# alasdairtran/transform-and-tell

Measured on AMD Instinct MI355X. Metric: training samples/sec (img+article->caption), higher is better.
Workload: dtype bf16; 1 GPU; BASELINE configs[2] (= per-GPU shape of configs[3]): expt/nytimes/9_transformer_objects - full faces+objects model (4 contexts: ResNet-152 image regions, RoBERTa-large article with the 25-layer weigh_bert mix, 4 faces, 64 objects), batch 32/GPU, 512-token articles, 32 caption steps; full step = frozen encoders fwd + decoder fwd/loss/bwd + BertAdam; global_batch=32, article_len=512, caption_len=33, parallelism=dp1, step_graph_replays=188, skipped_steps=0

## Files before the change

transform-and-tell_amd/csrc/common.h:

```cpp
#pragma once
#include <hip/hip_runtime.h>
#include <stdint.h>

#define TELL_OK 0
#define TELL_ERR_ARG (-1)
#define TELL_ERR_LAUNCH (-2)

#define TELL_F32 0
#define TELL_BF16 1

typedef __bf16 bf16_t;
typedef __attribute__((ext_vector_type(8))) __bf16 bf16x8;
typedef __attribute__((ext_vector_type(4))) float f32x4;
typedef __attribute__((ext_vector_type(16))) float f32x16;

extern "C" void tell_set_error(const char* msg);

static inline int tell_check_launch(const char* what) {
  hipError_t e = hipGetLastError();
  if (e != hipSuccess) {
    tell_set_error(hipGetErrorString(e));
    (void)what;
    return TELL_ERR_LAUNCH;
  }
  return TELL_OK;
}

#define TELL_REQUIRE(cond, msg)  \
  do {                           \
    if (!(cond)) {               \
      tell_set_error(msg);       \
      return TELL_ERR_ARG;       \
    }                            \
  } while (0)

__device__ __forceinline__ float bf2f(uint16_t b) { return __uint_as_float(((uint32_t)b) << 16); }
__device__ __forceinline__ uint16_t f2bf(float f) {
  uint32_t u = __float_as_uint(f);
  if ((u & 0x7fffffffu) > 0x7f800000u) return (uint16_t)((u >> 16) | 0x40u);
  u += 0x7fffu + ((u >> 16) & 1u);
  return (uint16_t)(u >> 16);
}

__device__ __forceinline__ float tell_glu(float a, float g) { return a * __builtin_amdgcn_rcpf(1.f + __expf(-g)); }

template <typename T> struct Elem;
template <> struct Elem<float> {
  static constexpr int VEC = 4;
  __device__ static __forceinline__ float ld(const float* p) { return *p; }
  __device__ static __forceinline__ void st(float* p, float v) { *p = v; }
};
template <> struct Elem<uint16_t> {
  static constexpr int VEC = 8;
  __device__ static __forceinline__ float ld(const uint16_t* p) { return bf2f(*p); }
  __device__ static __forceinline__ void st(uint16_t* p, float v) { *p = f2bf(v); }
};

__device__ __forceinline__ void unpack16(const uint4& c, float (&v)[4], const float*) {
  v[0] = __uint_as_float(c.x); v[1] = __uint_as_float(c.y);
  v[2] = __uint_as_float(c.z); v[3] = __uint_as_float(c.w);
}
__device__ __forceinline__ void unpack16(const uint4& c, float (&v)[8], const uint16_t*) {
  v[0] = __uint_as_float(c.x << 16); v[1] = __uint_as_float(c.x & 0xffff0000u);
  v[2] = __uint_as_float(c.y << 16); v[3] = __uint_as_float(c.y & 0xffff0000u);
  v[4] = __uint_as_float(c.z << 16); v[5] = __uint_as_float(c.z & 0xffff0000u);
  v[6] = __uint_as_float(c.w << 16); v[7] = __uint_as_float(c.w & 0xffff0000u);
}
__device__ __forceinline__ uint4 pack16(const float (&v)[4], const float*) {
  return make_uint4(__float_as_uint(v[0]), __float_as_uint(v[1]), __float_as_uint(v[2]),
                    __float_as_uint(v[3]));
}
__device__ __forceinline__ uint4 pack16(const float (&v)[8], const uint16_t*) {
  return make_uint4((uint32_t)f2bf(v[0]) | ((uint32_t)f2bf(v[1]) << 16),
                    (uint32_t)f2bf(v[2]) | ((uint32_t)f2bf(v[3]) << 16),
                    (uint32_t)f2bf(v[4]) | ((uint32_t)f2bf(v[5]) << 16),
                    (uint32_t)f2bf(v[6]) | ((uint32_t)f2bf(v[7]) << 16));
}

__device__ __forceinline__ float wave_sum(float v) {
#pragma unroll
  for (int o = 32; o > 0; o >>= 1) v += __shfl_xor(v, o, 64);
  return v;
}
__device__ __forceinline__ float wave_max(float v) {
#pragma unroll
  for (int o = 32; o > 0; o >>= 1) v = fmaxf(v, __shfl_xor(v, o, 64));
  return v;
}

extern const uint32_t* g_tell_rng_step;
extern const uint32_t* g_tell_pos_step;
extern uint32_t* g_tell_pos_next;
__device__ __forceinline__ uint32_t tell_step_salt(uint32_t salt, const uint32_t* step) {
  return step ? salt + *step * 0x632BE5ABu : salt;
}

__device__ __host__ __forceinline__ uint32_t tell_quad_x(uint32_t seed, uint64_t quad) {
  return (uint32_t)quad * 0x9E3779B1u + seed * 0x85EBCA6Bu;
}
__device__ __host__ __forceinline__ uint32_t tell_quad_y(uint32_t salt, uint64_t quad) {
  return (uint32_t)(quad >> 32) * 0x85EBCA77u + salt * 0xC2B2AE3Du + 0x27D4EB2Fu;
}
__device__ __host__ __forceinline__ uint32_t tell_quad_mix(uint32_t x, uint32_t y) {
  x ^= y; x ^= x >> 16; x *= 0x7FEB352Du; x ^= x >> 15;
  return x;
}
__device__ __host__ __forceinline__ uint32_t tell_quad_a(uint32_t h) {
  const uint32_t a = (h & 0xffffffu) * 0xD1B54Bu;
  return a ^ (a >> 15);
}
__device__ __host__ __forceinline__ uint32_t tell_quad_b(uint32_t h) {
  const uint32_t b = (h >> 8) * 0xA54FF5u;
  return b ^ (b >> 15);
}
__device__ __host__ __forceinline__ uint32_t tell_keep_field(uint32_t seed, uint32_t salt, uint64_t idx) {
  const uint64_t quad = idx >> 2;
  const uint32_t h = tell_quad_mix(tell_quad_x(seed, quad), tell_quad_y(salt, quad));
  const uint32_t w = (idx & 2) ? tell_quad_b(h) : tell_quad_a(h);
  return (idx & 1) ? (w >> 16) : (w & 0xffffu);
}
__device__ __host__ __forceinline__ uint32_t tell_drop_threshold(float p) {
  double t = (double)p * 65536.0;
  if (t < 0) t = 0;
  if (t > 65535.0) t = 65535.0;
  return (uint32_t)t;
}
__device__ __forceinline__ float tell_keep(uint32_t seed, uint32_t salt, uint64_t idx, uint32_t thr,
                                           float inv_keep) {
  return tell_keep_field(seed, salt, idx) >= thr ? inv_keep : 0.f;
}
__device__ __forceinline__ void tell_keep2(uint32_t seed, uint32_t salt, uint64_t idx_even, uint32_t thr,
                                           float inv_keep, float& k0, float& k1) {
  const uint64_t quad = idx_even >> 2;
  const uint32_t h = tell_quad_mix(tell_quad_x(seed, quad), tell_quad_y(salt, quad));
  const uint32_t w = (idx_even & 2) ? tell_quad_b(h) : tell_quad_a(h);
  k0 = (w & 0xffffu) >= thr ? inv_keep : 0.f;
  k1 = (w >> 16) >= thr ? inv_keep : 0.f;
}
struct TellKeepRow { uint32_t x0, y; };
#define TELL_QUAD_STRIDE 0x9E3779B1u
__device__ __forceinline__ bool tell_keep_row_ok(uint64_t quad0, uint32_t span) {
  return (uint32_t)quad0 <= 0xFFFFFFFFu - span;
}
__device__ __forceinline__ TellKeepRow tell_keep_row(uint32_t seed, uint32_t salt, uint64_t quad0) {
  TellKeepRow r;
  r.x0 = tell_quad_x(seed, quad0);
  r.y = tell_quad_y(salt, quad0);
  return r;
}
__device__ __forceinline__ void tell_keep4_bits(uint32_t x, uint32_t y, uint32_t thr, bool& k0, bool& k1, bool& k2,
                                                bool& k3) {
  const uint32_t h = tell_quad_mix(x, y);
  const uint32_t a = tell_quad_a(h), b = tell_quad_b(h);
  k0 = (a & 0xffffu) >= thr;
  k1 = (a >> 16) >= thr;
  k2 = (b & 0xffffu) >= thr;
  k3 = (b >> 16) >= thr;
}

__device__ __host__ __forceinline__ uint32_t tell_sample_bits(uint32_t seed, uint32_t row, uint32_t step) {
  const uint32_t h = tell_quad_mix(tell_quad_x(seed, row), tell_quad_y(step, row));
  return tell_quad_mix(h, 0x27D4EB2Fu);
}
__device__ __host__ __forceinline__ float tell_sample_u(uint32_t seed, uint32_t row, uint32_t step) {
  return (float)(tell_sample_bits(seed, row, step) >> 8) * (1.0f / 16777216.0f);
}
__device__ __host__ __forceinline__ int tell_sample_pick(const float* lp, int k, float inv_temp, float u) {
  const float l0 = lp[0];
  float c = 0.f;
  for (int j = 0; j < k; ++j) c += expf((lp[j] - l0) * inv_temp);
  const float t = u * c;
  float r = 0.f;
  for (int j = 0; j < k; ++j) {
    r += expf((lp[j] - l0) * inv_temp);
    if (t < r) return j;
  }
  return k - 1;
}
```

transform-and-tell_amd/csrc/elementwise.hip:

```cpp
#include "common.h"
#include "gemm_common.h"

static inline int grid_for(long work, int per_block) {
  long g = (work + per_block - 1) / per_block;
  if (g < 1) g = 1;
  if (g > 256 * 16) g = 256 * 16;
  return (int)g;
}

template <typename S, typename D>
__global__ void cast_kernel(const S* __restrict__ src, D* __restrict__ dst, long n) {
  long i = (long)blockIdx.x * blockDim.x + threadIdx.x;
  const long stride = (long)gridDim.x * blockDim.x;
  for (; i < n; i += stride) Elem<D>::st(dst + i, Elem<S>::ld(src + i));
}

extern "C" int tell_cast(const void* src, int src_dtype, void* dst, int dst_dtype, long n,
                         hipStream_t stream) {
  if (n <= 0) return TELL_OK;
  int g = grid_for(n, 256 * 4);
  if (src_dtype == TELL_F32 && dst_dtype == TELL_BF16)
    hipLaunchKernelGGL((cast_kernel<float, uint16_t>), dim3(g), dim3(256), 0, stream, (const float*)src, (uint16_t*)dst, n);
  else if (src_dtype == TELL_BF16 && dst_dtype == TELL_F32)
    hipLaunchKernelGGL((cast_kernel<uint16_t, float>), dim3(g), dim3(256), 0, stream, (const uint16_t*)src, (float*)dst, n);
  else if (src_dtype == TELL_F32 && dst_dtype == TELL_F32)
    hipLaunchKernelGGL((cast_kernel<float, float>), dim3(g), dim3(256), 0, stream, (const float*)src, (float*)dst, n);
  else if (src_dtype == TELL_BF16 && dst_dtype == TELL_BF16)
    hipLaunchKernelGGL((cast_kernel<uint16_t, uint16_t>), dim3(g), dim3(256), 0, stream, (const uint16_t*)src, (uint16_t*)dst, n);
  else { tell_set_error("cast: bad dtype"); return TELL_ERR_ARG; }
  return tell_check_launch("cast");
}

template <typename D>
__global__ __launch_bounds__(256) void scale_cast_kernel(const float* __restrict__ src, D* __restrict__ dst, long n,
                                                         const float* __restrict__ scale) {
  const float sc = scale ? *scale : 1.f;
  const long nv = n / 4;
  for (long i = (long)blockIdx.x * blockDim.x + threadIdx.x; i < nv; i += (long)gridDim.x * blockDim.x) {
    const float4 v = reinterpret_cast<const float4*>(src)[i];
    Elem<D>::st(dst + 4 * i, v.x * sc); Elem<D>::st(dst + 4 * i + 1, v.y * sc);
    Elem<D>::st(dst + 4 * i + 2, v.z * sc); Elem<D>::st(dst + 4 * i + 3, v.w * sc);
  }
  if (blockIdx.x == 0 && threadIdx.x < (n & 3)) Elem<D>::st(dst + nv * 4 + threadIdx.x, src[nv * 4 + threadIdx.x] * sc);
}
extern "C" int tell_scale_cast(const float* src, void* dst, int dst_dtype, long n, const float* scale_dev,
                               hipStream_t stream) {
  if (n <= 0) return TELL_OK;
  TELL_REQUIRE(((uintptr_t)src & 15) == 0, "scale_cast: src must be 16-byte aligned");
  int g = grid_for(n / 4 + 1, 256 * 2);
  if (dst_dtype == TELL_BF16) hipLaunchKernelGGL((scale_cast_kernel<uint16_t>), dim3(g), dim3(256), 0, stream, src, (uint16_t*)dst, n, scale_dev);
  else hipLaunchKernelGGL((scale_cast_kernel<float>), dim3(g), dim3(256), 0, stream, src, (float*)dst, n, scale_dev);
  return tell_check_launch("scale_cast");
}

template <typename S, typename D>
__global__ __launch_bounds__(256) void transpose_kernel(const S* __restrict__ src, long ld_src,
                                                        D* __restrict__ dst_t, long ld_t,
                                                        D* __restrict__ dst_plain, long ld_p,
                                                        const float* __restrict__ row_scale,
                                                        int rows, int cols) {
  __shared__ float tile[64][65];
  const int r0 = blockIdx.y * 64, c0 = blockIdx.x * 64;
  const int tx = threadIdx.x & 63, ty = threadIdx.x >> 6;
  for (int i = ty; i < 64; i += 4) {
    int r = r0 + i, c = c0 + tx;
    float v = 0.f;
    if (r < rows && c < cols) {
      v = Elem<S>::ld(src + (long)r * ld_src + c);
      if (row_scale) v *= row_scale[r];
      if (dst_plain) Elem<D>::st(dst_plain + (long)r * ld_p + c, v);
    }
    tile[i][tx] = v;
  }
  __syncthreads();
  if (dst_t) {
    for (int i = ty; i < 64; i += 4) {
      int c = c0 + i, r = r0 + tx;
      if (r < rows && c < cols) Elem<D>::st(dst_t + (long)c * ld_t + r, tile[tx][i]);
    }
  }
}

extern "C" int tell_transpose(const void* src, long ld_src, int src_dtype, void* dst_t, long ld_t,
                              void* dst_plain, long ld_p, int dst_dtype, const float* row_scale,
                              int rows, int cols, hipStream_t stream) {
  if (rows <= 0 || cols <= 0) return TELL_OK;
  dim3 grid((cols + 63) / 64, (rows + 63) / 64);
#define TL(S, D) hipLaunchKernelGGL((transpose_kernel<S, D>), grid, dim3(256), 0, stream, (const S*)src, ld_src, \
                                    (D*)dst_t, ld_t, (D*)dst_plain, ld_p, row_scale, rows, cols)
  if (src_dtype == TELL_F32 && dst_dtype == TELL_F32) TL(float, float);
  else if (src_dtype == TELL_F32 && dst_dtype == TELL_BF16) TL(float, uint16_t);
  else if (src_dtype == TELL_BF16 && dst_dtype == TELL_BF16) TL(uint16_t, uint16_t);
  else if (src_dtype == TELL_BF16 && dst_dtype == TELL_F32) TL(uint16_t, float);
  else { tell_set_error("transpose: bad dtype"); return TELL_ERR_ARG; }
#undef TL
  return tell_check_launch("transpose");
}

__global__ __launch_bounds__(256) void wn_rowscale_kernel(const float* __restrict__ g,
                                                          const float* __restrict__ v, int rows,
                                                          int cols, float* __restrict__ scale,
                                                          float* __restrict__ norms) {
  const int lane = threadIdx.x & 63;
  const int row = blockIdx.x * 4 + (threadIdx.x >> 6);
  if (row >= rows) return;
  const float* vr = v + (long)row * cols;
  float s = 0.f;
  for (int c = lane; c < cols; c += 64) { float x = vr[c]; s += x * x; }
  s = wave_sum(s);
  if (lane == 0) {
    float nrm = sqrtf(s);
    norms[row] = nrm;
    scale[row] = g[row] / nrm;
  }
}

extern "C" int tell_wn_rowscale(const float* g, const float* v, int rows, int cols, float* scale,
                                float* norms, hipStream_t stream) {
  if (rows <= 0) return TELL_OK;
  hipLaunchKernelGGL(wn_rowscale_kernel, dim3((rows + 3) / 4), dim3(256), 0, stream, g, v, rows, cols, scale, norms);
  return tell_check_launch("wn_rowscale");
}

template <typename OutT>
__device__ __forceinline__ void wn_weight_row(const float* __restrict__ g, const float* __restrict__ v, int row,
                                              int cols, OutT* __restrict__ w, float* __restrict__ norms, int lane) {
  const float* vr = v + (long)row * cols;
  OutT* wr = w + (long)row * cols;
  float s = 0.f;
  typedef __attribute__((ext_vector_type(4))) float f4v;
  if ((cols & 255) == 0 && cols <= 4096) {
    const int nv = cols >> 8;
    f4v x[16];
#pragma unroll
    for (int j = 0; j < 16; ++j)
      if (j < nv) x[j] = __builtin_nontemporal_load(reinterpret_cast<const f4v*>(vr) + lane + 64 * j);
#pragma unroll
    for (int j = 0; j < 16; ++j)
      if (j < nv) s += x[j][0] * x[j][0] + x[j][1] * x[j][1] + x[j][2] * x[j][2] + x[j][3] * x[j][3];
    s = wave_sum(s);
    const float nrm = sqrtf(s), sc = g[row] / nrm;
    if (lane == 0) norms[row] = nrm;
#pragma unroll
    for (int j = 0; j < 16; ++j)
      if (j < nv) {
        const int c = lane + 64 * j;
        if constexpr (sizeof(OutT) == 2) {
          uint2 o;
          o.x = (uint32_t)f2bf(x[j][0] * sc) | ((uint32_t)f2bf(x[j][1] * sc) << 16);
          o.y = (uint32_t)f2bf(x[j][2] * sc) | ((uint32_t)f2bf(x[j][3] * sc) << 16);
          reinterpret_cast<uint2*>(wr)[c] = o;
        } else {
          reinterpret_cast<float4*>(wr)[c] = make_float4(x[j][0] * sc, x[j][1] * sc, x[j][2] * sc, x[j][3] * sc);
        }
      }
    return;
  }
  if ((cols & 3) == 0) {
    const float4* v4 = reinterpret_cast<const float4*>(vr);
    for (int c = lane; c < cols / 4; c += 64) { const float4 x = v4[c]; s += x.x * x.x + x.y * x.y + x.z * x.z + x.w * x.w; }
  } else {
    for (int c = lane; c < cols; c += 64) { const float x = vr[c]; s += x * x; }
  }
  s = wave_sum(s);
  const float nrm = sqrtf(s), sc = g[row] / nrm;
  if (lane == 0) norms[row] = nrm;
  if ((cols & 3) == 0) {
    const float4* v4 = reinterpret_cast<const float4*>(vr);
    for (int c = lane; c < cols / 4; c += 64) {
      const float4 x = v4[c];
      if constexpr (sizeof(OutT) == 2) {
        uint2 o;
        o.x = (uint32_t)f2bf(x.x * sc) | ((uint32_t)f2bf(x.y * sc) << 16);
        o.y = (uint32_t)f2bf(x.z * sc) | ((uint32_t)f2bf(x.w * sc) << 16);
        reinterpret_cast<uint2*>(wr)[c] = o;
      } else {
        reinterpret_cast<float4*>(wr)[c] = make_float4(x.x * sc, x.y * sc, x.z * sc, x.w * sc);
      }
    }
  } else {
    for (int c = lane; c < cols; c += 64) Elem<OutT>::st(wr + c, vr[c] * sc);
  }
}
template <typename OutT>
__global__ __launch_bounds__(256) void wn_weight_kernel(const float* __restrict__ g, const float* __restrict__ v,
                                                        int rows, int cols, OutT* __restrict__ w,
                                                        float* __restrict__ norms) {
  const int row = blockIdx.x * 4 + (threadIdx.x >> 6);
  if (row < rows) wn_weight_row<OutT>(g, v, row, cols, w, norms, threadIdx.x & 63);
}
extern "C" int tell_wn_weight(const float* g, const float* v, int rows, int cols, void* w, int out_dtype,
                              float* norms, hipStream_t stream) {
  if (rows <= 0) return TELL_OK;
  TELL_REQUIRE(((uintptr_t)v & 15) == 0 && ((uintptr_t)w & 15) == 0, "wn_weight: buffers must be 16-byte aligned");
  if (out_dtype == TELL_BF16)
    hipLaunchKernelGGL((wn_weight_kernel<uint16_t>), dim3((rows + 3) / 4), dim3(256), 0, stream, g, v, rows, cols, (uint16_t*)w, norms);
  else
    hipLaunchKernelGGL((wn_weight_kernel<float>), dim3((rows + 3) / 4), dim3(256), 0, stream, g, v, rows, cols, (float*)w, norms);
  return tell_check_launch("wn_weight");
}

__device__ __forceinline__ void wn_backward_row(const float* __restrict__ dW, const float* __restrict__ g,
                                                const float* __restrict__ v, const float* __restrict__ norms,
                                                int row, int cols, float* __restrict__ dg, float* __restrict__ dv,
                                                int lane, const bool store = false) {
  const float* vr = v + (long)row * cols;
  const float* dr = dW + (long)row * cols;
  float* o = dv + (long)row * cols;
  const bool vec = (cols & 3) == 0 && (((uintptr_t)dW | (uintptr_t)v | (uintptr_t)dv) & 15) == 0;
  float dot = 0.f;
  if (vec && (cols & 255) == 0 && cols <= 4096) {
    typedef __attribute__((ext_vector_type(4))) float f4v;
    const int nv = cols >> 8;
    f4v d[16], x[16];
#pragma unroll
    for (int j = 0; j < 16; ++j)
      if (j < nv) {
        d[j] = __builtin_nontemporal_load(reinterpret_cast<const f4v*>(dr) + lane + 64 * j);
        x[j] = reinterpret_cast<const f4v*>(vr)[lane + 64 * j];
      }
#pragma unroll
    for (int j = 0; j < 16; ++j)
      if (j < nv) dot += d[j][0] * x[j][0] + d[j][1] * x[j][1] + d[j][2] * x[j][2] + d[j][3] * x[j][3];
    dot = wave_sum(dot);
    const float nrm = norms[row], gs = g[row] / nrm, k = dot / (nrm * nrm);
    if (lane == 0) dg[row] = (store ? 0.f : dg[row]) + dot / nrm;
#pragma unroll
    for (int j = 0; j < 16; ++j)
      if (j < nv) {
        const int c = lane + 64 * j;
        float4 a = make_float4(0.f, 0.f, 0.f, 0.f);
        if (!store) a = reinterpret_cast<float4*>(o)[c];
        a.x += gs * (d[j][0] - x[j][0] * k); a.y += gs * (d[j][1] - x[j][1] * k);
        a.z += gs * (d[j][2] - x[j][2] * k); a.w += gs * (d[j][3] - x[j][3] * k);
        reinterpret_cast<float4*>(o)[c] = a;
      }
    return;
  }
  if (vec) {
    for (int c = lane; c < cols / 4; c += 64) {
      const float4 d = reinterpret_cast<const float4*>(dr)[c], x = reinterpret_cast<const float4*>(vr)[c];
      dot += d.x * x.x + d.y * x.y + d.z * x.z + d.w * x.w;
    }
  } else {
    for (int c = lane; c < cols; c += 64) dot += dr[c] * vr[c];
  }
  dot = wave_sum(dot);
  const float nrm = norms[row], gs = g[row] / nrm, k = dot / (nrm * nrm);
  if (lane == 0) dg[row] = (store ? 0.f : dg[row]) + dot / nrm;
  if (vec) {
    for (int c = lane; c < cols / 4; c += 64) {
      const float4 d = reinterpret_cast<const float4*>(dr)[c], x = reinterpret_cast<const float4*>(vr)[c];
      float4 a = make_float4(0.f, 0.f, 0.f, 0.f);
      if (!store) a = reinterpret_cast<float4*>(o)[c];
      a.x += gs * (d.x - x.x * k); a.y += gs * (d.y - x.y * k); a.z += gs * (d.z - x.z * k); a.w += gs * (d.w - x.w * k);
      reinterpret_cast<float4*>(o)[c] = a;
    }
  } else {
    for (int c = lane; c < cols; c += 64) o[c] = (store ? 0.f : o[c]) + gs * (dr[c] - vr[c] * k);
  }
}
__global__ __launch_bounds__(256) void wn_backward_kernel(const float* __restrict__ dW,
                                                          const float* __restrict__ g,
                                                          const float* __restrict__ v,
                                                          const float* __restrict__ norms, int rows,
                                                          int cols, float* __restrict__ dg,
                                                          float* __restrict__ dv) {
  const int row = blockIdx.x * 4 + (threadIdx.x >> 6);
  if (row < rows) wn_backward_row(dW, g, v, norms, row, cols, dg, dv, threadIdx.x & 63);
}

extern "C" int tell_wn_backward(const float* dW, const float* g, const float* v, const float* norms,
                                int rows, int cols, float* dg, float* dv, hipStream_t stream) {
  if (rows <= 0) return TELL_OK;
  hipLaunchKernelGGL(wn_backward_kernel, dim3((rows + 3) / 4), dim3(256), 0, stream, dW, g, v, norms, rows, cols, dg, dv);
  return tell_check_launch("wn_backward");
}

#define WN_MULTI_MAX 32
struct WNMulti {
  const float* a[WN_MULTI_MAX];
  const float* g[WN_MULTI_MAX];
  const float* v[WN_MULTI_MAX];
  void* w[WN_MULTI_MAX];
  float* norms[WN_MULTI_MAX];
  float* dg[WN_MULTI_MAX];
  int cols[WN_MULTI_MAX];
  int row_start[WN_MULTI_MAX + 1];
  int n;
  unsigned store;
};
template <typename OutT, bool BWD>
__global__ __launch_bounds__(256) void wn_multi_kernel(WNMulti m) {
  const int row = blockIdx.x * 4 + (threadIdx.x >> 6), lane = threadIdx.x & 63;
  if (row >= m.row_start[m.n]) return;
  int i = 0;
  while (i + 1 < m.n && row >= m.row_start[i + 1]) ++i;
  const int r = row - m.row_start[i];
  if constexpr (BWD) wn_backward_row(m.a[i], m.g[i], m.v[i], m.norms[i], r, m.cols[i], m.dg[i], static_cast<float*>(m.w[i]), lane, (m.store >> i) & 1u);
  else wn_weight_row<OutT>(m.g[i], m.v[i], r, m.cols[i], static_cast<OutT*>(m.w[i]), m.norms[i], lane);
}
template <bool BWD>
static int wn_multi_launch(int n, const void* const* a, const void* const* g, const void* const* v, void* const* w,
                           void* const* norms, void* const* dg, const int* rows, const int* cols, int out_dtype,
                           hipStream_t stream, const int* store = nullptr) {
  static_assert(WN_MULTI_MAX <= 32, "WNMulti::store is one bit per tensor");
  for (int base = 0; base < n; base += WN_MULTI_MAX) {
    WNMulti m;
    m.n = n - base < WN_MULTI_MAX ? n - base : WN_MULTI_MAX;
    m.row_start[0] = 0;
    m.store = 0u;
    for (int i = 0; i < m.n; ++i) {
      const int j = base + i;
      TELL_REQUIRE(rows[j] > 0 && cols[j] > 0, "wn_multi: empty tensor");
      TELL_REQUIRE(BWD || (((uintptr_t)v[j] | (uintptr_t)w[j]) & 15) == 0, "wn_weight_multi: buffers must be 16-byte aligned");
      m.a[i] = BWD ? static_cast<const float*>(a[j]) : nullptr;
      m.g[i] = static_cast<const float*>(g[j]);
      m.v[i] = static_cast<const float*>(v[j]);
      m.w[i] = w[j];
      m.norms[i] = static_cast<float*>(norms[j]);
      m.dg[i] = BWD ? static_cast<float*>(dg[j]) : nullptr;
      m.cols[i] = cols[j];
      m.row_start[i + 1] = m.row_start[i] + rows[j];
      if (BWD && store && store[j]) m.store |= 1u << i;
    }
    const dim3 grid((m.row_start[m.n] + 3) / 4);
    if (BWD) hipLaunchKernelGGL((wn_multi_kernel<float, true>), grid, dim3(256), 0, stream, m);
    else if (out_dtype == TELL_BF16) hipLaunchKernelGGL((wn_multi_kernel<uint16_t, false>), grid, dim3(256), 0, stream, m);
    else hipLaunchKernelGGL((wn_multi_kernel<float, false>), grid, dim3(256), 0, stream, m);
  }
  return tell_check_launch(BWD ? "wn_backward_multi" : "wn_weight_multi");
}
extern "C" int tell_wn_weight_multi(int n, const void* const* g, const void* const* v, void* const* w,
                                    void* const* norms, const int* rows, const int* cols, int out_dtype,
                                    hipStream_t stream) {
  if (n <= 0) return TELL_OK;
  return wn_multi_launch<false>(n, nullptr, g, v, w, norms, nullptr, rows, cols, out_dtype, stream);
}
extern "C" int tell_wn_backward_multi(int n, const void* const* dW, const void* const* g, const void* const* v,
                                      const void* const* norms, const int* rows, const int* cols, void* const* dg,
                                      void* const* dv, hipStream_t stream) {
  if (n <= 0) return TELL_OK;
  return wn_multi_launch<true>(n, dW, g, v, dv, const_cast<void* const*>(norms), dg, rows, cols, TELL_F32, stream);
}
extern "C" int tell_wn_backward_multi2(int n, const void* const* dW, const void* const* g, const void* const* v,
                                       const void* const* norms, const int* rows, const int* cols, void* const* dg,
                                       void* const* dv, const int* store, hipStream_t stream) {
  if (n <= 0) return TELL_OK;
  return wn_multi_launch<true>(n, dW, g, v, dv, const_cast<void* const*>(norms), dg, rows, cols, TELL_F32, stream, store);
}

template <typename T>
__global__ void glu_fwd_kernel(const T* __restrict__ h, T* __restrict__ y, long rows, int C) {
  long i = (long)blockIdx.x * blockDim.x + threadIdx.x;
  const long n = rows * C, stride = (long)gridDim.x * blockDim.x;
  for (; i < n; i += stride) {
    long r = i / C; int c = (int)(i % C);
    float a = Elem<T>::ld(h + r * 2 * C + c), g = Elem<T>::ld(h + r * 2 * C + C + c);
    Elem<T>::st(y + i, tell_glu(a, g));
  }
}
template <typename T>
__global__ void glu_bwd_kernel(const T* __restrict__ h, const T* __restrict__ dy, T* __restrict__ dh,
                               long rows, int C) {
  long i = (long)blockIdx.x * blockDim.x + threadIdx.x;
  const long n = rows * C, stride = (long)gridDim.x * blockDim.x;
  for (; i < n; i += stride) {
    long r = i / C; int c = (int)(i % C);
    float a = Elem<T>::ld(h + r * 2 * C + c), g = Elem<T>::ld(h + r * 2 * C + C + c);
    float s = 1.f / (1.f + __expf(-g)), d = Elem<T>::ld(dy + i);
    Elem<T>::st(dh + r * 2 * C + c, d * s);
    Elem<T>::st(dh + r * 2 * C + C + c, d * a * s * (1.f - s));
  }
}
extern "C" int tell_glu_fwd(const void* h, void* y, long rows, int C, int dtype, hipStream_t stream) {
  if (rows <= 0) return TELL_OK;
  int g = grid_for(rows * C, 256 * 2);
  if (dtype == TELL_BF16) hipLaunchKernelGGL((glu_fwd_kernel<uint16_t>), dim3(g), dim3(256), 0, stream, (const uint16_t*)h, (uint16_t*)y, rows, C);
  else hipLaunchKernelGGL((glu_fwd_kernel<float>), dim3(g), dim3(256), 0, stream, (const float*)h, (float*)y, rows, C);
  return tell_check_launch("glu_fwd");
}
extern "C" int tell_glu_bwd(const void* h, const void* dy, void* dh, long rows, int C, int dtype,
                            hipStream_t stream) {
  if (rows <= 0) return TELL_OK;
  int g = grid_for(rows * C, 256 * 2);
  if (dtype == TELL_BF16) hipLaunchKernelGGL((glu_bwd_kernel<uint16_t>), dim3(g), dim3(256), 0, stream, (const uint16_t*)h, (const uint16_t*)dy, (uint16_t*)dh, rows, C);
  else hipLaunchKernelGGL((glu_bwd_kernel<float>), dim3(g), dim3(256), 0, stream, (const float*)h, (const float*)dy, (float*)dh, rows, C);
  return tell_check_launch("glu_bwd");
}

template <typename T>
__global__ void dropout_kernel(const T* __restrict__ x, T* __restrict__ y, long n, uint32_t thr,
                               float inv_keep, uint32_t seed, uint32_t salt,
                               const uint32_t* __restrict__ step) {
  salt = tell_step_salt(salt, step);
  long i = (long)blockIdx.x * blockDim.x + threadIdx.x;
  const long stride = (long)gridDim.x * blockDim.x;
  for (; i < n; i += stride)
    Elem<T>::st(y + i, Elem<T>::ld(x + i) * tell_keep(seed, salt, (uint64_t)i, thr, inv_keep));
}
extern "C" int tell_dropout(const void* x, void* y, long n, float p, uint32_t seed, uint32_t salt,
                            int dtype, hipStream_t stream) {
  if (n <= 0) return TELL_OK;
  TELL_REQUIRE(p >= 0.f && p < 1.f, "dropout: p must be in [0,1)");
  int g = grid_for(n, 256 * 4);
  uint32_t thr = tell_drop_threshold(p);
  float ik = 1.f / (1.f - p);
  if (dtype == TELL_BF16) hipLaunchKernelGGL((dropout_kernel<uint16_t>), dim3(g), dim3(256), 0, stream, (const uint16_t*)x, (uint16_t*)y, n, thr, ik, seed, salt, g_tell_rng_step);
  else hipLaunchKernelGGL((dropout_kernel<float>), dim3(g), dim3(256), 0, stream, (const float*)x, (float*)y, n, thr, ik, seed, salt, g_tell_rng_step);
  return tell_check_launch("dropout");
}

__global__ __launch_bounds__(256) void gelu_vec_kernel(const uint16_t* __restrict__ x, uint16_t* __restrict__ y, long nv) {
  for (long i = (long)blockIdx.x * blockDim.x + threadIdx.x; i < nv; i += (long)gridDim.x * blockDim.x) {
    const u32x4 v = *reinterpret_cast<const u32x4*>(x + i * 8);
    u32x4 o;
#pragma unroll
    for (int q = 0; q < 4; ++q) {
      const f32x2e_t r = gelu_erf2(f32x2e_t{__uint_as_float(v[q] << 16), __uint_as_float(v[q] & 0xffff0000u)});
      o[q] = pack2_bf16(r[0], r[1]);
    }
    *reinterpret_cast<u32x4*>(y + i * 8) = o;
  }
}
extern "C" int tell_gelu(const void* x, void* y, long n, int dtype, hipStream_t stream) {
  if (n <= 0) return TELL_OK;
  TELL_REQUIRE(dtype == TELL_BF16 && n % 8 == 0 && (((uintptr_t)x | (uintptr_t)y) & 15) == 0,
               "gelu: bf16, a multiple of 8 elements, 16-byte aligned buffers");
  const long nv = n / 8;
  const int g = (int)((nv + 255) / 256 > 16384 ? 16384 : (nv + 255) / 256);
  hipLaunchKernelGGL(gelu_vec_kernel, dim3(g), dim3(256), 0, stream, (const uint16_t*)x, (uint16_t*)y, nv);
  return tell_check_launch("gelu");
}

template <typename T>
__global__ __launch_bounds__(256) void colsum_partial_kernel(const T* __restrict__ x, long ld, int rows, int C,
                                                             int rows_per_chunk, float* __restrict__ partial,
                                                             const int* __restrict__ m_dev, float* __restrict__ direct,
                                                             int accumulate, float scale) {
  __shared__ float part[4][65];
  if (m_dev) { int md = *m_dev; rows = md < rows ? md : rows; }
  const int cx = threadIdx.x & 63, ry = threadIdx.x >> 6;
  const int c = blockIdx.x * 64 + cx;
  const int r0 = blockIdx.y * rows_per_chunk;
  const int r1 = r0 + rows_per_chunk < rows ? r0 + rows_per_chunk : rows;
  float s = 0.f;
  if (c < C)
    for (int r = r0 + ry; r < r1; r += 4) s += Elem<T>::ld(x + (long)r * ld + c);
  part[ry][cx] = s;
  __syncthreads();
  if (ry == 0 && c < C) {
    const float t = part[0][cx] + part[1][cx] + part[2][cx] + part[3][cx];
    if (direct) direct[c] = (accumulate ? direct[c] : 0.f) + scale * t;
    else partial[(long)blockIdx.y * C + c] = t;
  }
}
__global__ void colsum_finish_kernel(const float* __restrict__ partial, int n_chunks, int C, float* __restrict__ out,
                                     int accumulate, float scale) {
  const int c = blockIdx.x * blockDim.x + threadIdx.x;
  if (c >= C) return;
  float t = 0.f;
  for (int k = 0; k < n_chunks; ++k) t += partial[(long)k * C + c];
  t *= scale;
  out[c] = accumulate ? out[c] + t : t;
}
extern "C" int tell_colsum_chunks(int rows) { int n = (rows + 127) / 128; return n < 1 ? 1 : (n > 128 ? 128 : n); }
extern "C" int tell_colsum(const void* x, long ld, int rows, int C, int dtype, float* out,
                           int accumulate, const int* m_dev, float scale, float* workspace, hipStream_t stream) {
  if (C <= 0) return TELL_OK;
  const int nch = tell_colsum_chunks(rows);
  const int rpc = (rows + nch - 1) / nch;
  dim3 grid((C + 63) / 64, nch);
  float* direct = nch == 1 ? out : nullptr;
  if (dtype == TELL_BF16) hipLaunchKernelGGL((colsum_partial_kernel<uint16_t>), grid, dim3(256), 0, stream, (const uint16_t*)x, ld, rows, C, rpc, workspace, m_dev, direct, accumulate, scale);
  else hipLaunchKernelGGL((colsum_partial_kernel<float>), grid, dim3(256), 0, stream, (const float*)x, ld, rows, C, rpc, workspace, m_dev, direct, accumulate, scale);
  if (!direct) hipLaunchKernelGGL(colsum_finish_kernel, dim3((C + 255) / 256), dim3(256), 0, stream, workspace, nch, C, out, accumulate, scale);
  return tell_check_launch("colsum");
}

template <typename T>
__global__ void gather_rows_kernel(const T* __restrict__ src, long ld_src, const int* __restrict__ idx,
                                   const int* __restrict__ count_dev, int cap, T* __restrict__ dst,
                                   long ld_dst, int C) {
  int n = count_dev ? *count_dev : cap;
  if (n > cap) n = cap;
  for (int r = blockIdx.x; r < n; r += gridDim.x) {
    const T* s = src + (long)idx[r] * ld_src;
    T* d = dst + (long)r * ld_dst;
    for (int c = threadIdx.x; c < C; c += blockDim.x) d[c] = s[c];
  }
}
template <typename T>
__global__ void scatter_add_rows_kernel(const T* __restrict__ src, long ld_src, const int* __restrict__ idx,
                                        const int* __restrict__ count_dev, int cap, T* __restrict__ dst,
                                        long ld_dst, int C) {
  int n = count_dev ? *count_dev : cap;
  if (n > cap) n = cap;
  for (int r = blockIdx.x; r < n; r += gridDim.x) {
    const T* s = src + (long)r * ld_src;
    T* d = dst + (long)idx[r] * ld_dst;
    for (int c = threadIdx.x; c < C; c += blockDim.x)
      Elem<T>::st(d + c, Elem<T>::ld(d + c) + Elem<T>::ld(s + c));
  }
}
extern "C" int tell_gather_rows(const void* src, long ld_src, const int* idx, const int* count_dev,
                                int cap, void* dst, long ld_dst, int C, int dtype, hipStream_t stream) {
  if (cap <= 0) return TELL_OK;
  int g = cap < 2048 ? cap : 2048;
  if (dtype == TELL_BF16) hipLaunchKernelGGL((gather_rows_kernel<uint16_t>), dim3(g), dim3(256), 0, stream, (const uint16_t*)src, ld_src, idx, count_dev, cap, (uint16_t*)dst, ld_dst, C);
  else hipLaunchKernelGGL((gather_rows_kernel<float>), dim3(g), dim3(256), 0, stream, (const float*)src, ld_src, idx, count_dev, cap, (float*)dst, ld_dst, C);
  return tell_check_launch("gather_rows");
}
extern "C" int tell_scatter_add_rows(const void* src, long ld_src, const int* idx, const int* count_dev,
                                     int cap, void* dst, long ld_dst, int C, int dtype,
                                     hipStream_t stream) {
  if (cap <= 0) return TELL_OK;
  int g = cap < 2048 ? cap : 2048;
  if (dtype == TELL_BF16) hipLaunchKernelGGL((scatter_add_rows_kernel<uint16_t>), dim3(g), dim3(256), 0, stream, (const uint16_t*)src, ld_src, idx, count_dev, cap, (uint16_t*)dst, ld_dst, C);
  else hipLaunchKernelGGL((scatter_add_rows_kernel<float>), dim3(g), dim3(256), 0, stream, (const float*)src, ld_src, idx, count_dev, cap, (float*)dst, ld_dst, C);
  return tell_check_launch("scatter_add_rows");
}

template <typename D>
__global__ __launch_bounds__(256) void nan_rows_kernel(const float* __restrict__ x, int rows, int C,
                                                       D* __restrict__ y, uint8_t* __restrict__ mask) {
  const int lane = threadIdx.x & 63;
  const int row = blockIdx.x * 4 + (threadIdx.x >> 6);
  if (row >= rows) return;
  const float* xr = x + (long)row * C;
  int bad = 0;
  for (int c = lane; c < C; c += 64) bad |= (xr[c] != xr[c]);
  bad = __any(bad);
  if (lane == 0) mask[row] = bad ? 1 : 0;
  D* yr = y + (long)row * C;
  for (int c = lane; c < C; c += 64) Elem<D>::st(yr + c, bad ? 0.f : xr[c]);
}
extern "C" int tell_nan_rows(const float* x, int rows, int C, void* y, int out_dtype, uint8_t* mask,
                             hipStream_t stream) {
  if (rows <= 0) return TELL_OK;
  dim3 grid((rows + 3) / 4);
  if (out_dtype == TELL_BF16) hipLaunchKernelGGL((nan_rows_kernel<uint16_t>), grid, dim3(256), 0, stream, x, rows, C, (uint16_t*)y, mask);
  else hipLaunchKernelGGL((nan_rows_kernel<float>), grid, dim3(256), 0, stream, x, rows, C, (float*)y, mask);
  return tell_check_launch("nan_rows");
}

template <typename T>
__global__ __launch_bounds__(256) void mix_fwd_kernel(const T* __restrict__ H, const float* __restrict__ w,
                                                      int L, long n, T* __restrict__ out) {
  __shared__ float sw[64];
  if (threadIdx.x < 64) {
    float v = threadIdx.x < L ? w[threadIdx.x] : -INFINITY;
    float m = wave_max(v);
    float e = threadIdx.x < L ? __expf(v - m) : 0.f;
    float s = wave_sum(e);
    sw[threadIdx.x] = e / s;
  }
  __syncthreads();
  long i = (long)blockIdx.x * blockDim.x + threadIdx.x;
  const long stride = (long)gridDim.x * blockDim.x;
  for (; i < n; i += stride) {
    float acc = 0.f;
    for (int l = 0; l < L; ++l) acc += sw[l] * Elem<T>::ld(H + (long)l * n + i);
    Elem<T>::st(out + i, acc);
  }
}
template <typename T>
__global__ __launch_bounds__(256) void mix_bwd_kernel(const T* __restrict__ H, const T* __restrict__ dOut,
                                                      int L, long n, float* __restrict__ partial) {
  __shared__ float red[4][64];
  const int lane = threadIdx.x & 63, wave = threadIdx.x >> 6;
  for (int l = 0; l < L; ++l) {
    float acc = 0.f;
    for (long i = (long)blockIdx.x * blockDim.x + threadIdx.x; i < n; i += (long)gridDim.x * blockDim.x)
      acc += Elem<T>::ld(dOut + i) * Elem<T>::ld(H + (long)l * n + i);
    acc = wave_sum(acc);
    if (lane == 0) red[wave][l] = acc;
  }
  __syncthreads();
  if (threadIdx.x < L)
    partial[(long)blockIdx.x * L + threadIdx.x] =
        red[0][threadIdx.x] + red[1][threadIdx.x] + red[2][threadIdx.x] + red[3][threadIdx.x];
}
template <typename T>
__global__ __launch_bounds__(256) void mix_fwd_vec_kernel(const T* __restrict__ H, const float* __restrict__ w,
                                                          int L, long n, T* __restrict__ out) {
  constexpr int VEC = Elem<T>::VEC;
  __shared__ float sw[64];
  if (threadIdx.x < 64) {
    float v = threadIdx.x < L ? w[threadIdx.x] : -INFINITY;
    float m = wave_max(v);
    float e = threadIdx.x < L ? __expf(v - m) : 0.f;
    float s = wave_sum(e);
    sw[threadIdx.x] = e / s;
  }
  __syncthreads();
  const long nv = n / VEC;
  for (long i = (long)blockIdx.x * blockDim.x + threadIdx.x; i < nv; i += (long)gridDim.x * blockDim.x) {
    typedef __attribute__((ext_vector_type(4))) unsigned int u4;
    u4 hv[32];
#pragma unroll
    for (int l = 0; l < 32; ++l)
      if (l < L) hv[l] = __builtin_nontemporal_load(reinterpret_cast<const u4*>(H + (long)l * n + i * VEC));
    float acc[VEC];
#pragma unroll
    for (int k = 0; k < VEC; ++k) acc[k] = 0.f;
#pragma unroll
    for (int l = 0; l < 32; ++l)
      if (l < L) {
        float v[VEC];
        unpack16(make_uint4(hv[l][0], hv[l][1], hv[l][2], hv[l][3]), v, (const T*)nullptr);
        const float wl = sw[l];
#pragma unroll
        for (int k = 0; k < VEC; ++k) acc[k] += wl * v[k];
      }
    *reinterpret_cast<uint4*>(out + i * VEC) = pack16(acc, (const T*)nullptr);
  }
}
template <typename T>
__global__ __launch_bounds__(256) void mix_bwd_vec_kernel(const T* __restrict__ H, const T* __restrict__ dOut,
                                                          int L, long n, float* __restrict__ partial) {
  constexpr int VEC = Elem<T>::VEC;
  __shared__ float red[4][32];
  const int lane = threadIdx.x & 63, wave = threadIdx.x >> 6;
  float acc[32];
#pragma unroll
  for (int l = 0; l < 32; ++l) acc[l] = 0.f;
  const long nv = n / VEC;
  for (long i = (long)blockIdx.x * blockDim.x + threadIdx.x; i < nv; i += (long)gridDim.x * blockDim.x) {
    float d[VEC];
    unpack16(*reinterpret_cast<const uint4*>(dOut + i * VEC), d, (const T*)nullptr);
#pragma unroll
    for (int l = 0; l < 32; ++l) {
      if (l < L) {
        float v[VEC];
        unpack16(*reinterpret_cast<const uint4*>(H + (long)l * n + i * VEC), v, (const T*)nullptr);
        float a = acc[l];
#pragma unroll
        for (int k = 0; k < VEC; ++k) a += d[k] * v[k];
        acc[l] = a;
      }
    }
  }
#pragma unroll
  for (int l = 0; l < 32; ++l) {
    const float a = wave_sum(acc[l]);
    if (lane == 0) red[wave][l] = a;
  }
  __syncthreads();
  if (threadIdx.x < L)
    partial[(long)blockIdx.x * L + threadIdx.x] =
        red[0][threadIdx.x] + red[1][threadIdx.x] + red[2][threadIdx.x] + red[3][threadIdx.x];
}
extern "C" int tell_mix_fwd(const void* H, const float* w, int L, long n, void* out, int dtype,
                            hipStream_t stream) {
  TELL_REQUIRE(L >= 1 && L <= 64, "mix_fwd: L must be in [1,64]");
  if (L <= 32 && n % 8 == 0 && (((uintptr_t)H | (uintptr_t)out) & 15) == 0 && dtype == TELL_BF16) {
    hipLaunchKernelGGL((mix_fwd_vec_kernel<uint16_t>), dim3(grid_for(n / 8, 256)), dim3(256), 0, stream, (const uint16_t*)H, w, L, n, (uint16_t*)out);
    return tell_check_launch("mix_fwd_vec");
  }
  int g = grid_for(n, 256 * 4);
  if (dtype == TELL_BF16) hipLaunchKernelGGL((mix_fwd_kernel<uint16_t>), dim3(g), dim3(256), 0, stream, (const uint16_t*)H, w, L, n, (uint16_t*)out);
  else hipLaunchKernelGGL((mix_fwd_kernel<float>), dim3(g), dim3(256), 0, stream, (const float*)H, w, L, n, (float*)out);
  return tell_check_launch("mix_fwd");
}
extern "C" int tell_mix_bwd(const void* H, const void* dOut, int L, long n, float* partial,
                            int n_blocks, int dtype, hipStream_t stream) {
  TELL_REQUIRE(L >= 1 && L <= 64, "mix_bwd: L must be in [1,64]");
  TELL_REQUIRE(n_blocks >= 1, "mix_bwd: n_blocks");
  if (L <= 32 && n % 8 == 0 && (((uintptr_t)H | (uintptr_t)dOut) & 15) == 0 && dtype == TELL_BF16) {
    hipLaunchKernelGGL((mix_bwd_vec_kernel<uint16_t>), dim3(n_blocks), dim3(256), 0, stream, (const uint16_t*)H, (const uint16_t*)dOut, L, n, partial);
    return tell_check_launch("mix_bwd_vec");
  }
  if (dtype == TELL_BF16) hipLaunchKernelGGL((mix_bwd_kernel<uint16_t>), dim3(n_blocks), dim3(256), 0, stream, (const uint16_t*)H, (const uint16_t*)dOut, L, n, partial);
  else hipLaunchKernelGGL((mix_bwd_kernel<float>), dim3(n_blocks), dim3(256), 0, stream, (const float*)H, (const float*)dOut, L, n, partial);
  return tell_check_launch("mix_bwd");
}

__global__ __launch_bounds__(1024) void mix_wgrad_kernel(const float* __restrict__ partial, int n_blocks, int L,
                                                         const float* __restrict__ w, float* __restrict__ gw) {
  __shared__ float part[16][64];
  __shared__ float d[64], sm[64];
  const int t = threadIdx.x, l = t & 63, g = t >> 6;
  float s = 0.f;
  if (l < L)
    for (int b = g; b < n_blocks; b += 16) s += partial[(long)b * L + l];
  part[g][l] = s;
  __syncthreads();
  if (t < 64) {
    float v = 0.f;
#pragma unroll
    for (int q = 0; q < 16; ++q) v += part[q][t];
    d[t] = v;
  }
  float mx = -INFINITY;
  for (int j = 0; j < L; ++j) mx = fmaxf(mx, w[j]);
  float den = 0.f;
  for (int j = 0; j < L; ++j) den += __expf(w[j] - mx);
  if (t < L) sm[t] = __expf(w[t] - mx) / den;
  __syncthreads();
  float dot = 0.f;
  for (int j = 0; j < L; ++j) dot += sm[j] * d[j];
  if (t < L) gw[t] += sm[t] * (d[t] - dot);
}
extern "C" int tell_mix_wgrad(const float* partial, int n_blocks, int L, const float* w, float* gw, hipStream_t stream) {
  TELL_REQUIRE(L >= 1 && L <= 64 && n_blocks >= 1, "mix_wgrad: L must be in [1,64]");
  hipLaunchKernelGGL(mix_wgrad_kernel, dim3(1), dim3(1024), 0, stream, partial, n_blocks, L, w, gw);
  return tell_check_launch("mix_wgrad");
}

__global__ void loss_bits_kernel(const float* __restrict__ x, const int* __restrict__ n, float* __restrict__ out) {
  out[0] = x[0] / 0.69314718055994531f / (float)n[0];
}
extern "C" int tell_loss_bits(const float* x, const int* n_valid, float* out, hipStream_t stream) {
  hipLaunchKernelGGL(loss_bits_kernel, dim3(1), dim3(1), 0, stream, x, n_valid, out);
  return tell_check_launch("loss_bits");
}

template <typename T>
__global__ void axpy_kernel(const T* __restrict__ x, T* __restrict__ y, long n, float alpha) {
  long i = (long)blockIdx.x * blockDim.x + threadIdx.x;
  const long stride = (long)gridDim.x * blockDim.x;
  for (; i < n; i += stride) Elem<T>::st(y + i, Elem<T>::ld(y + i) + alpha * Elem<T>::ld(x + i));
}
extern "C" int tell_axpy(const void* x, void* y, long n, float alpha, int dtype, hipStream_t stream) {
  if (n <= 0) return TELL_OK;
  int g = grid_for(n, 256 * 4);
  if (dtype == TELL_BF16) hipLaunchKernelGGL((axpy_kernel<uint16_t>), dim3(g), dim3(256), 0, stream, (const uint16_t*)x, (uint16_t*)y, n, alpha);
  else hipLaunchKernelGGL((axpy_kernel<float>), dim3(g), dim3(256), 0, stream, (const float*)x, (float*)y, n, alpha);
  return tell_check_launch("axpy");
}

struct SumNArgs { const void* x[8]; };
template <typename T>
__global__ __launch_bounds__(256) void sum_n_kernel(SumNArgs a, int n_in, T* __restrict__ out, long n) {
  constexpr int VEC = Elem<T>::VEC;
  const long nv = n / VEC;
  for (long i = (long)blockIdx.x * blockDim.x + threadIdx.x; i < nv; i += (long)gridDim.x * blockDim.x) {
    float acc[VEC];
#pragma unroll
    for (int k = 0; k < VEC; ++k) acc[k] = 0.f;
#pragma unroll
    for (int j = 0; j < 8; ++j) {
      if (j < n_in) {
        float v[VEC];
        unpack16(*reinterpret_cast<const uint4*>(static_cast<const T*>(a.x[j]) + i * VEC), v, (const T*)nullptr);
#pragma unroll
        for (int k = 0; k < VEC; ++k) acc[k] += v[k];
      }
    }
    *reinterpret_cast<uint4*>(out + i * VEC) = pack16(acc, (const T*)nullptr);
  }
}
extern "C" int tell_sum_n(const void* x0, const void* x1, const void* x2, const void* x3, const void* x4,
                          const void* x5, const void* x6, const void* x7, int n_in, void* out, long n, int dtype,
                          hipStream_t stream) {
  if (n <= 0) return TELL_OK;
  const int vec = dtype == TELL_BF16 ? 8 : 4;
  TELL_REQUIRE(n_in >= 1 && n_in <= 8 && n % vec == 0, "sum_n: 1..8 inputs, n a multiple of one 16-byte chunk");
  SumNArgs a = {{x0, x1, x2, x3, x4, x5, x6, x7}};
  for (int j = 0; j < n_in; ++j) TELL_REQUIRE(a.x[j] && ((uintptr_t)a.x[j] & 15) == 0, "sum_n: inputs must be 16-byte aligned");
  int g = grid_for(n / vec, 256);
  if (dtype == TELL_BF16) hipLaunchKernelGGL((sum_n_kernel<uint16_t>), dim3(g), dim3(256), 0, stream, a, n_in, (uint16_t*)out, n);
  else hipLaunchKernelGGL((sum_n_kernel<float>), dim3(g), dim3(256), 0, stream, a, n_in, (float*)out, n);
  return tell_check_launch("sum_n");
}

template <typename T>
__global__ void relu_bwd_kernel(const T* __restrict__ dy, const T* __restrict__ y, T* __restrict__ dx, long n) {
  long i = (long)blockIdx.x * blockDim.x + threadIdx.x;
  const long stride = (long)gridDim.x * blockDim.x;
  for (; i < n; i += stride) Elem<T>::st(dx + i, Elem<T>::ld(y + i) > 0.f ? Elem<T>::ld(dy + i) : 0.f);
}
extern "C" int tell_relu_bwd(const void* dy, const void* y, void* dx, long n, int dtype, hipStream_t stream) {
  if (n <= 0) return TELL_OK;
  int g = grid_for(n, 256 * 4);
  if (dtype == TELL_BF16) hipLaunchKernelGGL((relu_bwd_kernel<uint16_t>), dim3(g), dim3(256), 0, stream, (const uint16_t*)dy, (const uint16_t*)y, (uint16_t*)dx, n);
  else hipLaunchKernelGGL((relu_bwd_kernel<float>), dim3(g), dim3(256), 0, stream, (const float*)dy, (const float*)y, (float*)dx, n);
  return tell_check_launch("relu_bwd");
}
```

transform-and-tell_amd/csrc/optim.hip:

```cpp
#include "common.h"
#include "options.h"

#define OPT_CHUNK 1024
#define TELL_ADAM_DEFAULT 4
#include <stdlib.h>
#include <type_traits>

__device__ __forceinline__ float4 load_grad4(const float* __restrict__ grad, const uint16_t* __restrict__ wire, long o) {
  if (wire) {
    const uint2 w = reinterpret_cast<const uint2*>(wire)[o];
    return make_float4(__uint_as_float(w.x << 16), __uint_as_float(w.x & 0xffff0000u), __uint_as_float(w.y << 16),
                       __uint_as_float(w.y & 0xffff0000u));
  }
  return reinterpret_cast<const float4*>(grad)[o];
}
template <int U>
__global__ __launch_bounds__(256) void sqsum_chunks_kernel(const float* __restrict__ grad, const uint16_t* __restrict__ wire,
                                                           long n_chunks, float grad_scale, float* __restrict__ partial) {
  __shared__ float red[U][4];
  for (long c0 = (long)blockIdx.x * U; c0 < n_chunks; c0 += (long)gridDim.x * U) {
    float4 g[U];
#pragma unroll
    for (int u = 0; u < U; ++u)
      g[u] = c0 + u < n_chunks ? load_grad4(grad, wire, (c0 + u) * OPT_CHUNK / 4 + threadIdx.x) : make_float4(0.f, 0.f, 0.f, 0.f);
#pragma unroll
    for (int u = 0; u < U; ++u) {
      float s = (g[u].x * g[u].x + g[u].y * g[u].y + g[u].z * g[u].z + g[u].w * g[u].w) * grad_scale * grad_scale;
      s = wave_sum(s);
      if ((threadIdx.x & 63) == 0) red[u][threadIdx.x >> 6] = s;
    }
    __syncthreads();
    if (threadIdx.x < U && c0 + threadIdx.x < n_chunks)
      partial[c0 + threadIdx.x] = red[threadIdx.x][0] + red[threadIdx.x][1] + red[threadIdx.x][2] + red[threadIdx.x][3];
    __syncthreads();
  }
}
__global__ __launch_bounds__(256) void tensor_norms_kernel(const float* __restrict__ partial,
                                                           const long* __restrict__ chunk_begin,
                                                           int n_tensors, float* __restrict__ norms,
                                                           int* __restrict__ skip) {
  __shared__ float red[4];
  const int t = blockIdx.x, lane = threadIdx.x & 63;
  const long c0 = chunk_begin[t], c1 = chunk_begin[t + 1];
  float s0 = 0.f, s1 = 0.f, s2 = 0.f, s3 = 0.f;
  long c = c0 + threadIdx.x;
  for (; c + 768 < c1; c += 1024) {
    s0 += partial[c]; s1 += partial[c + 256]; s2 += partial[c + 512]; s3 += partial[c + 768];
  }
  for (; c < c1; c += 256) s0 += partial[c];
  float s = wave_sum((s0 + s1) + (s2 + s3));
  if (lane == 0) red[threadIdx.x >> 6] = s;
  __syncthreads();
  if (threadIdx.x == 0) {
    s = (red[0] + red[1]) + (red[2] + red[3]);
    norms[t] = sqrtf(s);
    if (skip && !(fabsf(s) <= 3.4e38f)) atomicOr(skip, 2);
  }
}
__global__ void loss_flag_kernel(const float* __restrict__ loss, int* __restrict__ skip) {
  skip[0] = (fabsf(loss[0]) <= 3.4e38f) ? 0 : 1;
}
extern "C" int tell_loss_flag(const float* loss, int* skip, hipStream_t stream) {
  hipLaunchKernelGGL(loss_flag_kernel, dim3(1), dim3(1), 0, stream, loss, skip);
  return tell_check_launch("loss_flag");
}
__global__ void lr_schedule_kernel(const int* __restrict__ step, float lr, float warmup, float t_total,
                                   float* __restrict__ lr_dev) {
  double f = 1.0;
  if (t_total > 0.f) {
    const double x = (double)step[0] / (double)t_total, w = (double)warmup;
    f = x < w ? x / w : fmax((x - 1.0) / (w - 1.0), 0.0);
  }
  lr_dev[0] = (float)((double)lr * f);
}
#define TELL_ADAM_MAX_GROUPS 16
enum { HP_LR = 0, HP_WARMUP, HP_T_TOTAL, HP_B1, HP_B2, HP_EPS, HP_WD, HP_MAX_NORM, HP_COLS };
struct GroupTable {
  float row[TELL_ADAM_MAX_GROUPS][HP_COLS];
};
struct GroupArgs {
  const int* tensor_group;
  int n_groups;
  GroupTable hp;
};
__global__ void lr_schedule_groups_kernel(const int* __restrict__ step, GroupTable hp, int n_groups,
                                          float* __restrict__ lr_dev) {
  const int g = threadIdx.x;
  if (g >= n_groups) return;
  const float lr = hp.row[g][HP_LR], warmup = hp.row[g][HP_WARMUP], t_total = hp.row[g][HP_T_TOTAL];
  double f = 1.0;
  if (t_total > 0.f) {
    const double x = (double)step[0] / (double)t_total, w = (double)warmup;
    f = x < w ? x / w : fmax((x - 1.0) / (w - 1.0), 0.0);
  }
  lr_dev[g] = (float)((double)lr * f);
}
__global__ void ema_schedule_kernel(const int* __restrict__ step, float decay, float warm, float* __restrict__ omd_dev) {
  double d = (double)decay;
  if (step && warm > 0.f) {
    const double n = (double)step[0];
    d = fmin(d, (1.0 + n) / ((double)warm + n));
  }
  omd_dev[0] = (float)(1.0 - d);
}
struct EmaArgs {
  float* ema;
  const float* omd_dev;
};
template <typename T>
__device__ __forceinline__ const T* trailing_arg() { return nullptr; }
template <typename T, typename A, typename... R>
__device__ __forceinline__ const T* trailing_arg(const A& a, const R&... rest) {
  if constexpr (std::is_same<T, A>::value) return &a;
  else return trailing_arg<T>(rest...);
}
template <typename T, typename... Ts>
constexpr int count_of = (0 + ... + (std::is_same<T, Ts>::value ? 1 : 0));
template <int U, bool NT, typename... Ext>
__global__ __launch_bounds__(256) void bertadam_update_kernel(float* __restrict__ param,
                                                              float* __restrict__ grad,
                                                              float* __restrict__ m, float* __restrict__ v,
                                                              const int* __restrict__ chunk_tensor,
                                                              const float* __restrict__ norms, long n_chunks,
                                                              const float* __restrict__ lr_dev, float b1,
                                                              float b2, float eps, float wd, float max_norm,
                                                              float grad_scale, uint16_t* __restrict__ shadow,
                                                              int zero_grad, int* __restrict__ skip,
                                                              const uint16_t* __restrict__ wire,
                                                              int* __restrict__ step_dev,
                                                              const int* __restrict__ keep_grad, Ext... ext) {
  constexpr bool EMA = count_of<EmaArgs, Ext...> == 1, GROUPS = count_of<GroupArgs, Ext...> == 1;
  static_assert(sizeof...(Ext) == (EMA ? 1 : 0) + (GROUPS ? 1 : 0),
                "the optional trailing arguments are one EmaArgs, one GroupArgs, or both in that order");
  typedef __attribute__((ext_vector_type(4))) float f4;
  struct Hp { float lr, b1, b2, eps, wd, max_norm; };
  Hp one = {0.f, b1, b2, eps, wd, max_norm};
  if constexpr (!GROUPS) one.lr = *lr_dev;
  float* ema = nullptr;
  float omd = 0.f;
  if constexpr (EMA && !GROUPS) {
    const EmaArgs ea[] = {ext...};
    ema = ea[0].ema;
    omd = *ea[0].omd_dev;
  } else if constexpr (EMA) {
    const EmaArgs* ea = trailing_arg<EmaArgs>(ext...);
    ema = ea->ema;
    omd = *ea->omd_dev;
  }
  const GroupArgs* ga = nullptr;
  if constexpr (GROUPS) ga = trailing_arg<GroupArgs>(ext...);
  if (skip && skip[0] != 0) {
    if (blockIdx.x == 0 && threadIdx.x == 0) atomicAdd(skip + 1, 1);
    if (zero_grad)
      for (long c = blockIdx.x; c < n_chunks; c += gridDim.x)
        if (!keep_grad || !keep_grad[chunk_tensor[c]])
          reinterpret_cast<float4*>(grad)[c * OPT_CHUNK / 4 + threadIdx.x] = make_float4(0.f, 0.f, 0.f, 0.f);
    return;
  }
  if (step_dev && blockIdx.x == 0 && threadIdx.x == 0) atomicAdd(step_dev, 1);
  auto ldf = [](const float* base, long o) __attribute__((always_inline)) {
    const f4* q = reinterpret_cast<const f4*>(base) + o;
    return NT ? __builtin_nontemporal_load(q) : *q;
  };
  auto stf = [](float* base, long o, f4 val) __attribute__((always_inline)) {
    f4* q = reinterpret_cast<f4*>(base) + o;
    if (NT) __builtin_nontemporal_store(val, q); else *q = val;
  };
  for (long c0 = (long)blockIdx.x * U; c0 < n_chunks; c0 += (long)gridDim.x * U) {
    f4 g[U], p[U], mm[U], vv[U], e[EMA ? U : 1];
    float coef[U];
    int tensor[U], group[GROUPS ? U : 1];
    Hp hp[GROUPS ? U : 1];
#pragma unroll
    for (int u = 0; u < U; ++u) {
      const long c = c0 + u < n_chunks ? c0 + u : n_chunks - 1;
      const long o = c * OPT_CHUNK / 4 + threadIdx.x;
      if (wire) { const float4 w = load_grad4(grad, wire, o); g[u] = f4{w.x, w.y, w.z, w.w}; }
      else g[u] = ldf(grad, o);
      p[u] = ldf(param, o); mm[u] = ldf(m, o); vv[u] = ldf(v, o);
      if constexpr (EMA) e[u] = ldf(ema, o);
      tensor[u] = chunk_tensor[c];
      if constexpr (GROUPS) group[u] = ga->tensor_group[tensor[u]];
    }
#pragma unroll
    for (int u = 0; u < U; ++u) {
      if constexpr (GROUPS) {
        const int gi = (unsigned)group[u] < (unsigned)ga->n_groups ? group[u] : 0;
        const float* row = ga->hp.row[gi];
        hp[u] = Hp{lr_dev[gi], row[HP_B1], row[HP_B2], row[HP_EPS], row[HP_WD], row[HP_MAX_NORM]};
      }
      const float max_norm = GROUPS ? hp[GROUPS ? u : 0].max_norm : one.max_norm;
      coef[u] = grad_scale;
      if (max_norm > 0.f) {
        const float cc = max_norm / (norms[tensor[u]] + 1e-6f);
        if (cc < 1.f) coef[u] *= cc;
      }
    }
#pragma unroll
    for (int u = 0; u < U; ++u) {
      if (c0 + u >= n_chunks) break;
      const long o = (c0 + u) * OPT_CHUNK / 4 + threadIdx.x;
      const Hp h = GROUPS ? hp[GROUPS ? u : 0] : one;
      const float lr = h.lr, b1 = h.b1, b2 = h.b2, eps = h.eps, wd = h.wd;
#pragma unroll
      for (int k = 0; k < 4; ++k) {
#pragma clang fp contract(off)
        const float gg = g[u][k] * coef[u];
        mm[u][k] = __builtin_fmaf(1.f - b1, gg, b1 * mm[u][k]);
        const float g2 = ((1.f - b2) * gg) * gg;
        vv[u][k] = b2 * vv[u][k] + g2;
        p[u][k] = __builtin_fmaf(-lr, __builtin_fmaf(wd, p[u][k], mm[u][k] / (sqrtf(vv[u][k]) + eps)), p[u][k]);
        if constexpr (EMA) {
          const float d = p[u][k] - e[u][k];
          e[u][k] = __builtin_fmaf(omd, d, e[u][k]);
        }
      }
      stf(param, o, p[u]); stf(m, o, mm[u]); stf(v, o, vv[u]);
      if constexpr (EMA) stf(ema, o, e[u]);
      if (shadow) {
        uint2 sw;
        sw.x = (uint32_t)f2bf(p[u][0]) | ((uint32_t)f2bf(p[u][1]) << 16);
        sw.y = (uint32_t)f2bf(p[u][2]) | ((uint32_t)f2bf(p[u][3]) << 16);
        reinterpret_cast<uint2*>(shadow)[o] = sw;
      }
      if (zero_grad && !(keep_grad && keep_grad[tensor[u]])) stf(grad, o, f4{0.f, 0.f, 0.f, 0.f});
    }
  }
}

__global__ __launch_bounds__(256) void ema_swap_kernel(float* __restrict__ param, float* __restrict__ ema,
                                                       uint16_t* __restrict__ shadow, long n4) {
  typedef __attribute__((ext_vector_type(4))) float f4;
  for (long o = (long)blockIdx.x * 256 + threadIdx.x; o < n4; o += (long)gridDim.x * 256) {
    f4* pp = reinterpret_cast<f4*>(param) + o;
    f4* pe = reinterpret_cast<f4*>(ema) + o;
    const f4 p = __builtin_nontemporal_load(pp), e = __builtin_nontemporal_load(pe);
    __builtin_nontemporal_store(e, pp);
    __builtin_nontemporal_store(p, pe);
    if (shadow) {
      uint2 sw;
      sw.x = (uint32_t)f2bf(e[0]) | ((uint32_t)f2bf(e[1]) << 16);
      sw.y = (uint32_t)f2bf(e[2]) | ((uint32_t)f2bf(e[3]) << 16);
      reinterpret_cast<uint2*>(shadow)[o] = sw;
    }
  }
}
extern "C" int tell_ema_swap(float* param, float* ema, void* shadow_bf16, long n, hipStream_t stream) {
  TELL_REQUIRE(param && ema, "ema_swap: param and ema must not be NULL");
  TELL_REQUIRE(((uintptr_t)param & 15) == 0 && ((uintptr_t)ema & 15) == 0, "ema_swap: buffers must be 16-byte aligned");
  TELL_REQUIRE(((uintptr_t)shadow_bf16 & 7) == 0, "ema_swap: the bf16 shadow must be 8-byte aligned");
  TELL_REQUIRE(n >= 0 && n % OPT_CHUNK == 0, "ema_swap: n must be a whole number of chunks");
  if (n == 0) return TELL_OK;
  const long chunks = n / OPT_CHUNK;
  hipLaunchKernelGGL(ema_swap_kernel, dim3((int)(chunks < 8192 ? chunks : 8192)), dim3(256), 0, stream, param, ema,
                     (uint16_t*)shadow_bf16, n / 4);
  return tell_check_launch("ema_swap");
}

extern "C" int tell_opt_chunk(void) { return OPT_CHUNK; }

template <bool EMA>
static int bertadam_launch(float* param, float* grad, float* m, float* v, const int* chunk_tensor, const long* chunk_begin,
                           long n_chunks, int n_tensors, float* partial, float* norms, const float* lr_dev, float b1, float b2,
                           float eps, float wd, float max_norm, float grad_scale, void* shadow_bf16, int zero_grad, int* skip,
                           const void* grad_wire_bf16, int* step_dev, float lr_base, float warmup, float t_total,
                           const int* keep_grad, float* ema, float* omd_dev, float ema_decay, float ema_warm,
                           const GroupArgs* groups, hipStream_t stream) {
  if (n_chunks <= 0) return TELL_OK;
  if (EMA) {
    TELL_REQUIRE(ema && omd_dev, "bertadam: ema and ema_omd_dev must not be NULL");
    TELL_REQUIRE(((uintptr_t)ema & 15) == 0, "bertadam: ema must be 16-byte aligned");
    TELL_REQUIRE(ema_decay >= 0.f && ema_decay < 1.f, "bertadam: ema_decay must be in [0, 1)");
    TELL_REQUIRE(ema_warm >= 0.f && ema_warm <= 3.4e38f, "bertadam: ema_warm must be finite and not negative");
  }
  TELL_REQUIRE(((uintptr_t)grad_wire_bf16 & 7) == 0 && ((uintptr_t)shadow_bf16 & 7) == 0,
               "bertadam: the bf16 gradient and the bf16 shadow must be 8-byte aligned");
  const uint16_t* wire = static_cast<const uint16_t*>(grad_wire_bf16);
  TELL_REQUIRE(((uintptr_t)param & 15) == 0 && ((uintptr_t)grad & 15) == 0 && ((uintptr_t)m & 15) == 0 &&
                   ((uintptr_t)v & 15) == 0,
               "bertadam: buffers must be 16-byte aligned");
  if (groups) {
    max_norm = 0.f;
    for (int i = 0; i < groups->n_groups; ++i) {
      TELL_REQUIRE(groups->hp.row[i][HP_EPS] > 0.f, "bertadam: eps must be positive in every group");
      if (groups->hp.row[i][HP_MAX_NORM] > 0.f) max_norm = groups->hp.row[i][HP_MAX_NORM];
    }
  } else {
    TELL_REQUIRE(eps > 0.f, "bertadam: eps must be positive");
  }
  if (step_dev) {
    if (groups)
      hipLaunchKernelGGL(lr_schedule_groups_kernel, dim3(1), dim3(TELL_ADAM_MAX_GROUPS), 0, stream, step_dev, groups->hp,
                         groups->n_groups, const_cast<float*>(lr_dev));
    else
      hipLaunchKernelGGL(lr_schedule_kernel, dim3(1), dim3(1), 0, stream, step_dev, lr_base, warmup, t_total,
                         const_cast<float*>(lr_dev));
  }
  if (EMA) hipLaunchKernelGGL(ema_schedule_kernel, dim3(1), dim3(1), 0, stream, step_dev, ema_decay, ema_warm, omd_dev);
  const int var = tell_opt(OPT_ADAM_VAR) >= 0 ? (int)tell_opt(OPT_ADAM_VAR) : TELL_ADAM_DEFAULT;
  const int grid_env = tell_opt(OPT_ADAM_GRID) > 0 ? (int)tell_opt(OPT_ADAM_GRID) : 4096;
  const int U = (var == 1 || var == 3) ? 2 : (var == 2 || var == 4) ? 4 : 1;
  const long iters = (n_chunks + U - 1) / U;
  int g = iters < grid_env ? (int)iters : grid_env;
  if (max_norm > 0.f) {
    const long it4 = (n_chunks + 3) / 4;
    const int gs = it4 < 4096 ? (int)it4 : 4096;
    hipLaunchKernelGGL((sqsum_chunks_kernel<4>), dim3(gs), dim3(256), 0, stream, grad, wire, n_chunks, grad_scale, partial);
    hipLaunchKernelGGL(tensor_norms_kernel, dim3(n_tensors), dim3(256), 0, stream, partial, chunk_begin, n_tensors, norms, skip);
  }
#define TELL_ADAM_LAUNCH(UU, NTT)                                                                                               \
  do {                                                                                                                        \
    if (EMA && groups)                                                                                                        \
      hipLaunchKernelGGL((bertadam_update_kernel<UU, NTT, EmaArgs, GroupArgs>), dim3(g), dim3(256), 0, stream, param, grad, m,  \
                         v, chunk_tensor, norms, n_chunks, lr_dev, 0.f, 0.f, 0.f, 0.f, 0.f, grad_scale,                        \
                         (uint16_t*)shadow_bf16, zero_grad, skip, wire, step_dev, keep_grad, EmaArgs{ema, omd_dev}, *groups);  \
    else if (groups)                                                                                                          \
      hipLaunchKernelGGL((bertadam_update_kernel<UU, NTT, GroupArgs>), dim3(g), dim3(256), 0, stream, param, grad, m, v,        \
                         chunk_tensor, norms, n_chunks, lr_dev, 0.f, 0.f, 0.f, 0.f, 0.f, grad_scale,                          \
                         (uint16_t*)shadow_bf16, zero_grad, skip, wire, step_dev, keep_grad, *groups);                         \
    else if (EMA)                                                                                                             \
      hipLaunchKernelGGL((bertadam_update_kernel<UU, NTT, EmaArgs>), dim3(g), dim3(256), 0, stream, param, grad, m, v,              \
                         chunk_tensor, norms, n_chunks, lr_dev, b1, b2, eps, wd, max_norm, grad_scale,                        \
                         (uint16_t*)shadow_bf16, zero_grad, skip, wire, step_dev, keep_grad, EmaArgs{ema, omd_dev});           \
    else                                                                                                                      \
      hipLaunchKernelGGL((bertadam_update_kernel<UU, NTT>), dim3(g), dim3(256), 0, stream, param, grad, m, v, chunk_tensor,   \
                         norms, n_chunks, lr_dev, b1, b2, eps, wd, max_norm, grad_scale, (uint16_t*)shadow_bf16, zero_grad,   \
                         skip, wire, step_dev, keep_grad);                                                                    \
  } while (0)
  switch (var) {
    case 1: TELL_ADAM_LAUNCH(2, false); break;
    case 2: TELL_ADAM_LAUNCH(4, false); break;
    case 3: TELL_ADAM_LAUNCH(2, true); break;
    case 4: TELL_ADAM_LAUNCH(4, true); break;
    default: TELL_ADAM_LAUNCH(1, false); break;
  }
#undef TELL_ADAM_LAUNCH
  return tell_check_launch("bertadam_step");
}
extern "C" int tell_bertadam_step2(float* param, float* grad, float* m, float* v,
                                   const int* chunk_tensor, const long* chunk_begin, long n_chunks,
                                   int n_tensors, float* partial, float* norms, const float* lr_dev,
                                   float b1, float b2, float eps, float wd, float max_norm,
                                   float grad_scale, void* shadow_bf16, int zero_grad, int* skip,
                                   const void* grad_wire_bf16, int* step_dev, float lr_base, float warmup, float t_total,
                                   const int* keep_grad, hipStream_t stream) {
  return bertadam_launch<false>(param, grad, m, v, chunk_tensor, chunk_begin, n_chunks, n_tensors, partial, norms, lr_dev, b1,
                                b2, eps, wd, max_norm, grad_scale, shadow_bf16, zero_grad, skip, grad_wire_bf16, step_dev,
                                lr_base, warmup, t_total, keep_grad, nullptr, nullptr, 0.f, 0.f, nullptr, stream);
}
extern "C" int tell_bertadam_step_ema(float* param, float* grad, float* m, float* v,
                                      const int* chunk_tensor, const long* chunk_begin, long n_chunks,
                                      int n_tensors, float* partial, float* norms, const float* lr_dev,
                                      float b1, float b2, float eps, float wd, float max_norm,
                                      float grad_scale, void* shadow_bf16, int zero_grad, int* skip,
                                      const void* grad_wire_bf16, int* step_dev, float lr_base, float warmup, float t_total,
                                      const int* keep_grad, float* ema, float* ema_omd_dev, float ema_decay, float ema_warm,
                                      hipStream_t stream) {
  return bertadam_launch<true>(param, grad, m, v, chunk_tensor, chunk_begin, n_chunks, n_tensors, partial, norms, lr_dev, b1,
                               b2, eps, wd, max_norm, grad_scale, shadow_bf16, zero_grad, skip, grad_wire_bf16, step_dev,
                               lr_base, warmup, t_total, keep_grad, ema, ema_omd_dev, ema_decay, ema_warm, nullptr, stream);
}
extern "C" int tell_bertadam_step_groups(float* param, float* grad, float* m, float* v, const int* chunk_tensor,
                                         const long* chunk_begin, long n_chunks, int n_tensors, float* partial, float* norms,
                                         float* lr_dev, const int* tensor_group, const float* group_hp, int n_groups,
                                         float grad_scale, void* shadow_bf16, int zero_grad, int* skip,
                                         const void* grad_wire_bf16, int* step_dev, const int* keep_grad, float* ema,
                                         float* ema_omd_dev, float ema_decay, float ema_warm, hipStream_t stream) {
  if (n_chunks <= 0) return TELL_OK;
  TELL_REQUIRE(n_groups >= 1 && n_groups <= TELL_ADAM_MAX_GROUPS, "bertadam: n_groups must be in 1..16");
  TELL_REQUIRE(tensor_group && group_hp && lr_dev, "bertadam: tensor_group, group_hp and lr_dev must not be NULL");
  TELL_REQUIRE((ema == nullptr) == (ema_omd_dev == nullptr), "bertadam: ema and ema_omd_dev must be given together");
  GroupArgs ga = {};
  ga.tensor_group = tensor_group;
  ga.n_groups = n_groups;
  for (int i = 0; i < n_groups * HP_COLS; ++i) ga.hp.row[i / HP_COLS][i % HP_COLS] = group_hp[i];
  if (ema)
    return bertadam_launch<true>(param, grad, m, v, chunk_tensor, chunk_begin, n_chunks, n_tensors, partial, norms, lr_dev,
                                 0.f, 0.f, 0.f, 0.f, 0.f, grad_scale, shadow_bf16, zero_grad, skip, grad_wire_bf16, step_dev,
                                 0.f, 0.f, 0.f, keep_grad, ema, ema_omd_dev, ema_decay, ema_warm, &ga, stream);
  return bertadam_launch<false>(param, grad, m, v, chunk_tensor, chunk_begin, n_chunks, n_tensors, partial, norms, lr_dev, 0.f,
                                0.f, 0.f, 0.f, 0.f, grad_scale, shadow_bf16, zero_grad, skip, grad_wire_bf16, step_dev, 0.f,
                                0.f, 0.f, keep_grad, nullptr, nullptr, 0.f, 0.f, &ga, stream);
}
extern "C" int tell_bertadam_step(float* param, float* grad, float* m, float* v,
                                  const int* chunk_tensor, const long* chunk_begin, long n_chunks,
                                  int n_tensors, float* partial, float* norms, const float* lr_dev,
                                  float b1, float b2, float eps, float wd, float max_norm,
                                  float grad_scale, void* shadow_bf16, int zero_grad, int* skip,
                                  const void* grad_wire_bf16, int* step_dev, float lr_base, float warmup, float t_total,
                                  hipStream_t stream) {
  return tell_bertadam_step2(param, grad, m, v, chunk_tensor, chunk_begin, n_chunks, n_tensors, partial, norms, lr_dev, b1, b2,
                             eps, wd, max_norm, grad_scale, shadow_bf16, zero_grad, skip, grad_wire_bf16, step_dev, lr_base,
                             warmup, t_total, nullptr, stream);
}

__global__ void fill_kernel(float* __restrict__ x, long n, float value) {
  long i = (long)blockIdx.x * blockDim.x + threadIdx.x;
  const long stride = (long)gridDim.x * blockDim.x;
  for (; i < n; i += stride) x[i] = value;
}
extern "C" int tell_fill_f32(float* x, long n, float value, hipStream_t stream) {
  if (n <= 0) return TELL_OK;
  long g = (n + 1023) / 1024;
  if (g > 4096) g = 4096;
  hipLaunchKernelGGL(fill_kernel, dim3((int)g), dim3(256), 0, stream, x, n, value);
  return tell_check_launch("fill_f32");
}
```

transform-and-tell_amd/csrc/options.h:

```cpp
#pragma once
#include <atomic>

#define TELL_OPTION_LIST(X)                                                                                             \
                                  \
  X(OPT_GEMM_Q4, "gemm_q4", 1)                               \
  X(OPT_GEMM_Q4E, "gemm_q4e", 1)                         \
  X(OPT_Q4_PARTIAL, "q4_partial", 1)                                                 \
  X(OPT_Q4_DYNAMIC, "q4_dynamic", 0)        \
  X(OPT_Q4_VAR, "q4_var", 0)                \
  X(OPT_GEMM_PP2, "gemm_pp2", 2)                \
  X(OPT_PP2_DYNAMIC, "pp2_dynamic", 1)                                                                                  \
  X(OPT_PP2_GRID, "pp2_grid", 0)                          \
  X(OPT_GEMM_PERSIST, "gemm_persist", 0)                                                                                \
  X(OPT_GEMM_TILE, "gemm_tile", 0)          \
                                                                \
  X(OPT_GEMM_S64, "gemm_s64", 1)                                \
  X(OPT_GEMM_SMALL, "gemm_small", 1)                                                                                    \
  X(OPT_GEMM_RING, "gemm_ring", 0)               \
  X(OPT_GEMM_SPLITK, "gemm_splitk", -1)                                                                                 \
  X(OPT_GROUP_TILE, "group_tile", 0)                                                                                    \
  X(OPT_GROUP_WIDE, "group_wide", 1)                                                                                    \
  X(OPT_GROUP_SORT, "group_sort", 1)                                                                                    \
  X(OPT_CONV_TILE, "conv_tile", 0)                  \
  X(OPT_BN_FUSE, "bn_fuse", 1)                                                                                          \
  X(OPT_BN_COMBINE, "bn_combine", 0)                                                                                    \
  X(OPT_BN_WGS, "bn_wgs", 768)                                                                                          \
                                  \
  X(OPT_ATTN_TILE64, "attn_tile64", 0)                                                                                  \
  X(OPT_ATTN_SELF, "attn_self", 1)                                                                                      \
  X(OPT_ATTN_DMA, "attn_dma", 0)                                                                                        \
  X(OPT_ATTN_OCC, "attn_occ", 2)                                                                                        \
  X(OPT_DYNCONV_LDS, "dynconv_lds", 1)                                                                                  \
  X(OPT_DYNCONV_BLOCK, "dynconv_block", 1)                                                                              \
  X(OPT_LN_VAR, "ln_var", -1)                                                            \
  X(OPT_ARGMAX_REGS, "argmax_regs", 1)                                                                                  \
  X(OPT_ADAM_VAR, "adam_var", -1)                                                   \
  X(OPT_ADAM_GRID, "adam_grid", 4096)                                                                                   \
  X(OPT_SK_ROWS, "sk_rows", 0)              \
  X(OPT_SK_SPLIT, "sk_split", 0)            \
  X(OPT_SK_TALL_WAVES, "sk_tall_waves", 4)                    \
  X(OPT_SK_STAGED, "sk_staged", 1)

#define TELL_PROBE_LIST(X)                                                                                              \
  X(PROBE_Q4_ABL, "q4_abl", 0)                     \
  X(PROBE_Q4E_VAR, "q4e_var", -1)                                                      \
  X(PROBE_PP2_ABL, "pp2_abl", 0)                                                                                        \
  X(PROBE_DCB_ABL, "dcb_abl", 0)                                                                                        \
  X(PROBE_SK_STAMP_PTR, "sk_stamp_ptr", 0)        \
  X(PROBE_SK_STAMP_SLOTS, "sk_stamp_slots", 0)

enum TellOpt {
#define TELL_X(e, k, d) e,
  TELL_OPTION_LIST(TELL_X)
#ifdef TELL_PROBES
  TELL_PROBE_LIST(TELL_X)
#endif
#undef TELL_X
  TELL_OPT_COUNT
};

extern std::atomic<long> g_tell_opt[TELL_OPT_COUNT];
static inline long tell_opt(int o) { return g_tell_opt[o].load(std::memory_order_relaxed); }
#ifdef TELL_PROBES
#define tell_probe(e) tell_opt(e)
#else
#define tell_probe(e) 0L
#endif
```

transform-and-tell_amd/training/trainer.py:

```python
import contextlib
import os

import torch

from .. import hip, ops, streams
from .. import runtime as rt
from ..common.registrable import Registrable
from . import dp
from .optimizers import BertAdam, FlatParams, apply_no_grad


class TrainerBase(Registrable):
    pass


class Trainer:
    def __init__(self, model, optimizer_cfg=None, no_grad=(r'^resnet', r'^roberta'), device='cuda',
                 nan_check=False, bucket_mb=256, async_update=None, allreduce_dtype=None, data_parallel=None,
                 capture_after=None, shape_buckets=(128, 16)):
        import torch.distributed as dist
        self.dist = dist if (dist.is_available() and dist.is_initialized() and data_parallel is not False) else None
        self.world = self.dist.get_world_size() if self.dist else 1
        self.dp = self.world > 1 or (self.dist is not None and os.environ.get('TELL_DP_SELFTEST') == '1')
        self.rank = self.dist.get_rank() if self.dist else 0
        self.model = model.to(device)
        apply_no_grad(model, no_grad)
        if hasattr(model, 'reset_graphs'):
            model.reset_graphs()
        self.flat = FlatParams(model.named_parameters(), device)
        cfg = dict(lr=1e-4, warmup=0.05, t_total=437600, schedule='warmup_linear', b1=0.9, b2=0.98, e=1e-6,
                   weight_decay=1e-5, max_grad_norm=0.1)
        cfg.update(optimizer_cfg or {})
        cfg.pop('type', None)
        self.optimizer = BertAdam(self.flat, **cfg)
        self.nan_check = nan_check
        self.bucket_elems = bucket_mb * (1 << 20) // 4
        self.batch_num_total = 0
        if allreduce_dtype is None:
            allreduce_dtype = torch.bfloat16 if (rt.compute_dtype() == torch.bfloat16 and
                                                 torch.device(device).type == 'cuda' and
                                                 os.environ.get('TELL_ALLREDUCE_FP32') != '1') else torch.float32
        self.allreduce_dtype, self._wire = allreduce_dtype, None
        if self.dp and self.world > 1:
            if 'TELL_Q4_DYNAMIC' not in os.environ:
                hip.set_option('q4_dynamic', 1)
        if self.dp:
            rt.set_rank(self.rank)
        if self.dp:
            self.dist.broadcast(self.flat.flat, src=0)
            self.flat.refresh_shadow()
            rt.bump_weights_epoch()
        if self.optimizer.ema_decay is not None:
            self.optimizer.reset_ema()
        if async_update is None:
            async_update = os.environ.get('TELL_ASYNC_UPDATE', '0') == '1'
        self.async_update = async_update and torch.device(device).type == 'cuda'
        self.update_stream = streams.get('update', device) if self.async_update else None
        self.flat.zero_grad()
        self._stored_last = False
        self._store = 'want' if (torch.device(device).type == 'cuda' and
                                 os.environ.get('TELL_GRAD_STORE', '1') != '0') else 'off'
        self.model.register_state_dict_pre_hook(lambda *a, **k: self.finish_update())
        self._ranges, self._reduced, self._pending, self._in_backward = {}, [], [], False
        self._capturing = False
        self.defer_update = False
        on_gpu = torch.device(device).type == 'cuda'
        self.skip = torch.zeros(2, dtype=torch.int32, device=device) if on_gpu else None
        from .step_graph import StepGraph
        self.step_graph = StepGraph(self, capture_after) if on_gpu else None
        self.shape_buckets = tuple(shape_buckets) if shape_buckets else None
        if capture_after is not None and hasattr(model, 'set_capture_after'):
            model.set_capture_after(capture_after)
        self.bucketed_reduces = 0
        self.dp_timing = None
        self._test_reduce_scale = None
        from . import step_graph as _sg
        bucketed_default = '0' if (_sg.ENABLED and on_gpu) else '1'
        if self.dp and on_gpu and os.environ.get('TELL_DP_BUCKETED', bucketed_default) != '0':
            self._ranges = self._layer_ranges()
            if self._ranges:
                rt.set_grad_ready_callback(self._grad_ready)
                self.step_graph = None

    def _layer_ranges(self):
        fl, out = self.flat, {}
        ends = fl.offsets[1:] + [fl.total]
        for i in range(len(getattr(getattr(self.model, 'decoder', None), 'layers', []))):
            pre = 'decoder.layers.%d.' % i
            idx = [k for k, n in enumerate(fl.names) if n.startswith(pre)]
            if not idx or idx != list(range(idx[0], idx[-1] + 1)):
                return {}
            out[pre] = (fl.offsets[idx[0]], ends[idx[-1]])
        return out

    def _grad_ready(self, tag):
        rng_ = self._ranges.get(tag)
        if rng_ is None or not self._in_backward or self._capturing:
            return
        side = ops.flush_wgrad_stream()
        if side is not None:
            torch.cuda.current_stream().wait_stream(side)
        with hip.bound_stream():
            self._start_reduce(*rng_)
        self._reduced.append(rng_)
        self.bucketed_reduces += 1

    def dp_times(self):
        out = [(e[0].elapsed_time(e[2]), e[1].elapsed_time(e[2])) for e in (self.dp_timing or [])]
        if self.dp_timing is not None:
            self.dp_timing = []
        return out

    def finish_update(self):
        rt.wait_weight_update()

    def _swap_ema(self):
        f = self.flat
        with hip.bound_stream():
            hip.call('tell_ema_swap', f.flat, f.ema, f.shadow, f.total)
        self.optimizer.ema_swapped = not self.optimizer.ema_swapped
        rt.bump_weights_epoch()

    @contextlib.contextmanager
    def ema_weights(self):
        if self.optimizer.ema_decay is None:
            raise ValueError('Trainer.ema_weights() needs the optimizer option ema_decay (got ema_decay=None)')
        if self.optimizer.ema_swapped:
            raise RuntimeError('Trainer.ema_weights() does not nest')
        self.finish_update()
        self._swap_ema()
        try:
            yield self
        finally:
            self._swap_ema()

    def ema_state_dict(self):
        with self.ema_weights():
            return {k: v.detach().clone() for k, v in self.model.state_dict().items()}

    def train_one_batch(self, batch, next_batch=None):
        if self.optimizer.ema_swapped:
            raise RuntimeError('train_one_batch inside Trainer.ema_weights(): the masters sit in the EMA buffer')
        with hip.bound_stream():
            return self._train_one_batch(batch, next_batch)

    def _encoded_for(self, batch):
        pre, self._prefetched = getattr(self, '_prefetched', None), None
        if pre is not None and pre[0] is batch.get('image') and not pre[1].stale():
            return pre[1]
        return None

    def _bucketed(self, batch):
        from . import step_graph as _sg
        from .. import graphs
        if self.shape_buckets is None or not (_sg.ENABLED and graphs.ENABLED) or self.nan_check:
            return batch
        if not getattr(self.model, 'SHAPE_BUCKETS', True):
            return batch
        idx = getattr(self.model, 'index', 'roberta')
        pad = int(getattr(self.model, 'padding_idx', 1))
        out = None

        def grow(t, dim, n, value):
            shape = list(t.shape)
            shape[dim] = n - t.shape[dim]
            return torch.cat([t, t.new_full(shape, value)], dim=dim)
        for key, mult, extra in (('context', self.shape_buckets[0], 0), ('caption', self.shape_buckets[1], 1)):
            field = batch.get(key)
            ids = field.get(idx) if isinstance(field, dict) else None
            if not (torch.is_tensor(ids) and ids.is_cuda and ids.dim() == 2):
                continue
            n = -(-(ids.shape[1] - extra) // mult) * mult + extra
            if n != ids.shape[1]:
                out = dict(batch) if out is None else out
                f = dict(field)
                f[idx] = grow(ids, 1, n, pad)
                for mk in (idx + '_copy_masks', idx + '_proper_masks'):
                    m = f.get(mk)
                    if torch.is_tensor(m) and m.dim() == 2 and m.shape[1] == ids.shape[1]:
                        f[mk] = grow(m, 1, n, -1)
                out[key] = f
        for key, rows in (('face_embeds', 4), ('obj_embeds', 64)):
            t = batch.get(key)
            if torch.is_tensor(t) and t.is_cuda and t.dim() == 3 and t.shape[2] > 0 and t.shape[1] < rows:
                out = dict(batch) if out is None else out
                out[key] = grow(t, 1, rows, float('nan'))
        return batch if out is None else out

    @staticmethod
    def _store_safe(batch):
        for key in ('face_embeds', 'obj_embeds'):
            t = batch.get(key) if isinstance(batch, dict) else None
            if torch.is_tensor(t) and t.dim() == 3 and (t.shape[1] == 0 or t.shape[2] == 0):
                return False
        return True

    def _grad_store_begin(self, batch=None):
        want = (self._store == 'ready' and not self.defer_update and not self.flat.accum_pending and
                (batch is None or self._store_safe(batch)))
        if self._stored_last and not want:
            pending = self.flat.accum_pending
            self.flat.zero_grad()
            self.flat.accum_pending = pending
        self._stored_last = want
        ops.grad_store_mode(want)
        if self.defer_update:
            self.flat.accum_pending = True

    def _train_one_batch(self, batch, next_batch=None):
        try:
            return self._train_one_batch_body(batch, next_batch)
        finally:
            ops.grad_store_mode(False)

    def _train_one_batch_body(self, batch, next_batch=None):
        if not self.model.training:
            self.model.train()
        batch = self._bucketed(batch)
        self._grad_store_begin(batch)
        if next_batch is not None:
            next_batch = self._bucketed(next_batch)
        enc = None
        if hasattr(self.model, 'encode') and torch.is_tensor(batch.get('image')) and batch['image'].is_cuda:
            enc = self._encoded_for(batch)
            if enc is None:
                enc = self.model.encode(batch['context'], batch['image'])
            if next_batch is not None:
                self._prefetched = (next_batch['image'],
                                    self.model.encode(next_batch['context'], next_batch['image'], ahead=True))
        loss = None
        if enc is not None and self.step_graph is not None and not self.nan_check:
            loss = self.step_graph.run(batch, enc, self._eager_step)
        if loss is None:
            loss = self._eager_step(batch, enc)
        if loss is not None:
            self.batch_num_total += 1
        return loss

    def _flag_loss(self, loss):
        if loss.is_cuda:
            hip.call('tell_loss_flag', loss.detach().reshape(1).float(), self.skip)

    def _backward(self, scaled):
        self._in_backward = True
        ops.wn_defer(not self._ranges)
        ops.wgrad_group_defer(not self._ranges)
        ops.finish_defer(not self._ranges)
        observe = self._store == 'want' and not self._capturing
        if observe:
            ops.grad_store_observe(True)
        try:
            scaled.backward()
        except BaseException:
            ops.wn_drop()
            ops.wgrad_group_drop()
            ops.finish_drop()
            if observe:
                ops.grad_store_observe(False)
            raise
        finally:
            self._in_backward = False
            ops.wn_defer(False)
            ops.wgrad_group_defer(False)
            ops.finish_defer(False)
        ops.join_wgrad_stream()
        ops.wgrad_group_flush()
        ops.wn_flush()
        ops.finish_flush()
        if observe:
            self.flat.set_grad_store(ops.grad_store_observe(False))
            self._store = 'ready'
            self._stored_last = not self.defer_update
            ops.grad_store_mode(self._stored_last)

    def skipped_steps(self):
        return int(self.skip[1].item()) if self.skip is not None else 0

    def _eager_step(self, batch, enc=None):
        extra = {'encoded': enc} if enc is not None else {}
        out = self.model(**batch, **extra)
        loss = out['loss']
        if loss is None:
            return None
        self._flag_loss(loss)
        n_local = None
        if self.dp and self._ranges:
            scaled = loss * dp.loss_weight(out['sample_size'].to(torch.float32).reshape(1), self.dist,
                                           self.world).reshape(())
        else:
            scaled = loss
            n_local = out['sample_size'] if self.dp else None
        if self.nan_check:
            bad = (~torch.isfinite(loss.detach())).to(torch.float32)
            if self.dp:
                self.dist.all_reduce(bad)
            if bad.item() > 0:
                self.flat.zero_grad()
                return None
        self._backward(scaled)
        if self.async_update:
            main = torch.cuda.current_stream()
            self.update_stream.wait_stream(main)
            with torch.cuda.stream(self.update_stream), hip.bound_stream():
                self._update(n_local)
                done = torch.cuda.Event()
                done.record(self.update_stream)
            rt.set_pending_update(done)
        else:
            self._update(n_local)
        return loss.detach()

    def _update(self, n_local=None):
        if self.defer_update:
            return
        if self.dp:
            scale = None
            ev = None
            if self.dp_timing is not None and self.flat.grad.is_cuda:
                ev = [torch.cuda.Event(enable_timing=True) for _ in range(3)]
                ev[0].record()
            if n_local is not None:
                scale = dp.loss_weight(n_local.to(torch.float32).reshape(1), self.dist, self.world)
            if self.skip is not None and self.skip.is_cuda:
                self.dist.all_reduce(self.skip[:1], op=self.dist.ReduceOp.MAX)
            done, self._reduced = sorted(self._reduced), []
            lo = 0
            for a, b in done + [(self.flat.total, self.flat.total)]:
                if a > lo:
                    self._start_reduce(lo, a, scale)
                lo = max(lo, b)
            if ev is not None:
                ev[1].record()
            wire = self._finish_reduces()
            if ev is not None:
                ev[2].record()
                self.dp_timing.append(ev)
            if wire is not None:
                self.optimizer.step(grad_scale=1.0 / self.world, zero_grad=True, skip=self.skip, grad_wire=wire)
                return
        self.optimizer.step(grad_scale=1.0 / self.world, zero_grad=True, skip=self.skip)

    def _cast(self, src, dst):
        hip.call('tell_cast', src, hip.dt(src), dst, hip.dt(dst), src.numel())

    def _start_reduce(self, lo, hi, scale=None):
        grad = self.flat.grad[lo:hi]
        if self.allreduce_dtype == torch.bfloat16:
            if self._wire is None:
                self._wire = torch.empty(self.flat.total, dtype=torch.bfloat16, device=self.flat.grad.device)
            buf, step = self._wire[lo:hi], 2 * self.bucket_elems
            hip.call('tell_scale_cast', grad, buf, hip.BF16, grad.numel(), scale)
        else:
            buf, step = grad, self.bucket_elems
            if scale is not None:
                if grad.is_cuda:
                    hip.call('tell_scale_cast', grad, grad, hip.F32, grad.numel(), scale)
                else:
                    grad.mul_(scale)
        handles = [self.dist.all_reduce(buf[s:s + step], async_op=True) for s in range(0, buf.numel(), step)]
        self._pending.append((lo, hi, handles))

    def _finish_reduces(self):
        pending, self._pending = self._pending, []
        for lo, hi, handles in pending:
            for h in handles:
                h.wait()
        direct = (self.allreduce_dtype == torch.bfloat16 and self._test_reduce_scale is None and
                  self.flat.grad.is_cuda and len(pending) == 1 and pending[0][0] == 0 and
                  pending[0][1] == self.flat.total and hasattr(self.optimizer, 'launch'))
        if direct:
            return self._wire
        for lo, hi, handles in pending:
            grad = self.flat.grad[lo:hi]
            if self.allreduce_dtype == torch.bfloat16:
                self._cast(self._wire[lo:hi], grad)
            if self._test_reduce_scale is not None:
                grad.mul_(self._test_reduce_scale)
        return None


@TrainerBase.register('callback_apex')
class CallbackApexTrainer(Trainer):

    def __init__(self, model, optimizer=None, no_grad=(r'^resnet', r'^roberta'), apex_opt_level=None,
                 keep_batchnorm_fp32=None, num_epochs=1, shuffle=True, cuda_device=0, callbacks=None, **kw):
        super().__init__(model, optimizer, no_grad, device='cuda' if cuda_device is not None else 'cpu')
        self.num_epochs = num_epochs

    def train(self, batches):
        losses = []
        for batch in batches:
            losses.append(self.train_one_batch(batch))
        return losses
```

Measured before the change: 1641 samples/s.

## Run bandwidth-bound kernels on a few persistent workgroups when overlapping steps

Adds 'narrow' persistent variants of the weight-norm, layer-mix forward/backward, grad sqsum and BertAdam kernels. Each variant uses large workgroups and reserves 96KB of dynamic LDS so that only a capped number of workgroups (bw_wgs) occupy CUs, and each workgroup loops over virtual blocks. The trainer enables bw_wgs=128 and q4_dynamic only when a next batch is being prefetched. The intent is to leave CUs free for concurrent work, such as next-batch encoding, instead of letting these memory-bound kernels flood the device. The risk is that the throttled kernels run slower when nothing actually overlaps with them.

```diff
diff --git a/transform-and-tell_amd/csrc/common.h b/transform-and-tell_amd/csrc/common.h
--- a/transform-and-tell_amd/csrc/common.h
+++ b/transform-and-tell_amd/csrc/common.h
@@ -33,6 +33,18 @@
       return TELL_ERR_ARG;       \
     }                            \
   } while (0)
+
+#define TELL_NARROW_LDS (96 * 1024)
+template <typename... KA, typename... A>
+static inline void tell_launch_narrow(void (*kern)(KA...), long wgs, int threads, hipStream_t stream, A... args) {
+  (void)hipFuncSetAttribute(reinterpret_cast<const void*>(kern), hipFuncAttributeMaxDynamicSharedMemorySize, TELL_NARROW_LDS);
+  hipLaunchKernelGGL(kern, dim3((unsigned)(wgs < 1 ? 1 : wgs)), dim3(threads), TELL_NARROW_LDS, stream, args...);
+}
+__device__ __forceinline__ int tell_quarter() { return __builtin_amdgcn_readfirstlane((int)(threadIdx.x >> 8)); }
+static inline long tell_narrow_wgs(long G, long virtual_blocks, int per_wg = 4) {
+  const long need = (virtual_blocks + per_wg - 1) / per_wg;
+  return G < need ? G : need;
+}
 
 __device__ __forceinline__ float bf2f(uint16_t b) { return __uint_as_float(((uint32_t)b) << 16); }
 __device__ __forceinline__ uint16_t f2bf(float f) {
diff --git a/transform-and-tell_amd/csrc/elementwise.hip b/transform-and-tell_amd/csrc/elementwise.hip
--- a/transform-and-tell_amd/csrc/elementwise.hip
+++ b/transform-and-tell_amd/csrc/elementwise.hip
@@ -1,5 +1,6 @@
 #include "common.h"
 #include "gemm_common.h"
+#include "options.h"
 
 static inline int grid_for(long work, int per_block) {
   long g = (work + per_block - 1) / per_block;
@@ -291,14 +292,25 @@
   unsigned store;
 };
 template <typename OutT, bool BWD>
-__global__ __launch_bounds__(256) void wn_multi_kernel(WNMulti m) {
-  const int row = blockIdx.x * 4 + (threadIdx.x >> 6), lane = threadIdx.x & 63;
-  if (row >= m.row_start[m.n]) return;
+__device__ __forceinline__ void wn_multi_row(const WNMulti& m, int row, int lane) {
   int i = 0;
   while (i + 1 < m.n && row >= m.row_start[i + 1]) ++i;
   const int r = row - m.row_start[i];
   if constexpr (BWD) wn_backward_row(m.a[i], m.g[i], m.v[i], m.norms[i], r, m.cols[i], m.dg[i], static_cast<float*>(m.w[i]), lane, (m.store >> i) & 1u);
   else wn_weight_row<OutT>(m.g[i], m.v[i], r, m.cols[i], static_cast<OutT*>(m.w[i]), m.norms[i], lane);
+}
+template <typename OutT, bool BWD>
+__global__ __launch_bounds__(256) void wn_multi_kernel(WNMulti m) {
+  const int row = blockIdx.x * 4 + (threadIdx.x >> 6), lane = threadIdx.x & 63;
+  if (row >= m.row_start[m.n]) return;
+  wn_multi_row<OutT, BWD>(m, row, lane);
+}
+template <typename OutT, bool BWD, int THREADS>
+__global__ __launch_bounds__(THREADS) void wn_multi_narrow_kernel(WNMulti m) {
+  constexpr int W = THREADS / 64;
+  const int wave = __builtin_amdgcn_readfirstlane((int)(threadIdx.x >> 6)), lane = threadIdx.x & 63;
+  for (long row = (long)blockIdx.x * W + wave; row < m.row_start[m.n]; row += (long)gridDim.x * W)
+    wn_multi_row<OutT, BWD>(m, (int)row, lane);
 }
 template <bool BWD>
 static int wn_multi_launch(int n, const void* const* a, const void* const* g, const void* const* v, void* const* w,
@@ -325,7 +337,13 @@
       if (BWD && store && store[j]) m.store |= 1u << i;
     }
     const dim3 grid((m.row_start[m.n] + 3) / 4);
-    if (BWD) hipLaunchKernelGGL((wn_multi_kernel<float, true>), grid, dim3(256), 0, stream, m);
+    const long G = tell_opt(OPT_BW_WGS);
+    if (G > 0) {
+      const int total = m.row_start[m.n];
+      if (BWD) tell_launch_narrow(wn_multi_narrow_kernel<float, true, 512>, tell_narrow_wgs(G, total, 8), 512, stream, m);
+      else if (out_dtype == TELL_BF16) tell_launch_narrow(wn_multi_narrow_kernel<uint16_t, false, 1024>, tell_narrow_wgs(G, total, 16), 1024, stream, m);
+      else tell_launch_narrow(wn_multi_narrow_kernel<float, false, 1024>, tell_narrow_wgs(G, total, 16), 1024, stream, m);
+    } else if (BWD) hipLaunchKernelGGL((wn_multi_kernel<float, true>), grid, dim3(256), 0, stream, m);
     else if (out_dtype == TELL_BF16) hipLaunchKernelGGL((wn_multi_kernel<uint16_t, false>), grid, dim3(256), 0, stream, m);
     else hipLaunchKernelGGL((wn_multi_kernel<float, false>), grid, dim3(256), 0, stream, m);
   }
@@ -545,9 +563,8 @@
 }
 
 template <typename T>
-__global__ __launch_bounds__(256) void mix_fwd_kernel(const T* __restrict__ H, const float* __restrict__ w,
-                                                      int L, long n, T* __restrict__ out) {
-  __shared__ float sw[64];
+__device__ __forceinline__ void mix_fwd_body(const T* __restrict__ H, const float* __restrict__ w, int L, long n,
+                                             T* __restrict__ out, float* sw) {
   if (threadIdx.x < 64) {
     float v = threadIdx.x < L ? w[threadIdx.x] : -INFINITY;
     float m = wave_max(v);
@@ -565,27 +582,52 @@
   }
 }
 template <typename T>
+__global__ __launch_bounds__(256) void mix_fwd_kernel(const T* __restrict__ H, const float* __restrict__ w,
+                                                      int L, long n, T* __restrict__ out) {
+  __shared__ float sw[64];
+  mix_fwd_body<T>(H, w, L, n, out, sw);
+}
+template <typename T>
+__global__ __launch_bounds__(1024) void mix_fwd_narrow_kernel(const T* __restrict__ H, const float* __restrict__ w,
+                                                              int L, long n, T* __restrict__ out) {
+  __shared__ float sw[64];
+  mix_fwd_body<T>(H, w, L, n, out, sw);
+}
+template <typename T>
+__device__ __forceinline__ void mix_bwd_block(const T* __restrict__ H, const T* __restrict__ dOut, int L, long n,
+                                              float* __restrict__ partial, long b, long nb, int tid, bool active,
+                                              float (*red)[64]) {
+  const int lane = tid & 63, wave = tid >> 6;
+  for (int l = 0; l < L; ++l) {
+    float acc = 0.f;
+    for (long i = active ? b * 256 + tid : n; i < n; i += nb * 256)
+      acc += Elem<T>::ld(dOut + i) * Elem<T>::ld(H + (long)l * n + i);
+    acc = wave_sum(acc);
+    if (lane == 0) red[wave][l] = acc;
+  }
+  __syncthreads();
+  if (active && tid < L) partial[b * L + tid] = red[0][tid] + red[1][tid] + red[2][tid] + red[3][tid];
+}
+template <typename T>
 __global__ __launch_bounds__(256) void mix_bwd_kernel(const T* __restrict__ H, const T* __restrict__ dOut,
                                                       int L, long n, float* __restrict__ partial) {
   __shared__ float red[4][64];
-  const int lane = threadIdx.x & 63, wave = threadIdx.x >> 6;
-  for (int l = 0; l < L; ++l) {
-    float acc = 0.f;
-    for (long i = (long)blockIdx.x * blockDim.x + threadIdx.x; i < n; i += (long)gridDim.x * blockDim.x)
-      acc += Elem<T>::ld(dOut + i) * Elem<T>::ld(H + (long)l * n + i);
-    acc = wave_sum(acc);
-    if (lane == 0) red[wave][l] = acc;
-  }
-  __syncthreads();
-  if (threadIdx.x < L)
-    partial[(long)blockIdx.x * L + threadIdx.x] =
-        red[0][threadIdx.x] + red[1][threadIdx.x] + red[2][threadIdx.x] + red[3][threadIdx.x];
-}
-template <typename T>
-__global__ __launch_bounds__(256) void mix_fwd_vec_kernel(const T* __restrict__ H, const float* __restrict__ w,
-                                                          int L, long n, T* __restrict__ out) {
+  mix_bwd_block<T>(H, dOut, L, n, partial, blockIdx.x, gridDim.x, threadIdx.x, true, red);
+}
+template <typename T>
+__global__ __launch_bounds__(1024) void mix_bwd_narrow_kernel(const T* __restrict__ H, const T* __restrict__ dOut,
+                                                              int L, long n, float* __restrict__ partial, long nvb) {
+  __shared__ float red[4][4][64];
+  const int q = tell_quarter();
+  for (long vb0 = (long)blockIdx.x * 4; vb0 < nvb; vb0 += (long)gridDim.x * 4) {
+    mix_bwd_block<T>(H, dOut, L, n, partial, vb0 + q, nvb, threadIdx.x & 255, vb0 + q < nvb, red[q]);
+    __syncthreads();
+  }
+}
+template <typename T, int LB>
+__device__ __forceinline__ void mix_fwd_vec_body(const T* __restrict__ H, const float* __restrict__ w, int L, long n,
+                                                 T* __restrict__ out, float* sw) {
   constexpr int VEC = Elem<T>::VEC;
-  __shared__ float sw[64];
   if (threadIdx.x < 64) {
     float v = threadIdx.x < L ? w[threadIdx.x] : -INFINITY;
     float m = wave_max(v);
@@ -597,36 +639,51 @@
   const long nv = n / VEC;
   for (long i = (long)blockIdx.x * blockDim.x + threadIdx.x; i < nv; i += (long)gridDim.x * blockDim.x) {
     typedef __attribute__((ext_vector_type(4))) unsigned int u4;
-    u4 hv[32];
-#pragma unroll
-    for (int l = 0; l < 32; ++l)
-      if (l < L) hv[l] = __builtin_nontemporal_load(reinterpret_cast<const u4*>(H + (long)l * n + i * VEC));
     float acc[VEC];
 #pragma unroll
     for (int k = 0; k < VEC; ++k) acc[k] = 0.f;
 #pragma unroll
-    for (int l = 0; l < 32; ++l)
-      if (l < L) {
-        float v[VEC];
-        unpack16(make_uint4(hv[l][0], hv[l][1], hv[l][2], hv[l][3]), v, (const T*)nullptr);
-        const float wl = sw[l];
-#pragma unroll
-        for (int k = 0; k < VEC; ++k) acc[k] += wl * v[k];
-      }
+    for (int l0 = 0; l0 < 32; l0 += LB) {
+      u4 hv[LB];
+#pragma unroll
+      for (int l = 0; l < LB; ++l)
+        if (l0 + l < L) hv[l] = __builtin_nontemporal_load(reinterpret_cast<const u4*>(H + (long)(l0 + l) * n + i * VEC));
+#pragma unroll
+      for (int l = 0; l < LB; ++l)
+        if (l0 + l < L) {
+          float v[VEC];
+          unpack16(make_uint4(hv[l][0], hv[l][1], hv[l][2], hv[l][3]), v, (const T*)nullptr);
+          const float wl = sw[l0 + l];
+#pragma unroll
+          for (int k = 0; k < VEC; ++k) acc[k] += wl * v[k];
+        }
+    }
     *reinterpret_cast<uint4*>(out + i * VEC) = pack16(acc, (const T*)nullptr);
   }
 }
 template <typename T>
-__global__ __launch_bounds__(256) void mix_bwd_vec_kernel(const T* __restrict__ H, const T* __restrict__ dOut,
-                                                          int L, long n, float* __restrict__ partial) {
+__global__ __launch_bounds__(256) void mix_fwd_vec_kernel(const T* __restrict__ H, const float* __restrict__ w,
+                                                          int L, long n, T* __restrict__ out) {
+  __shared__ float sw[64];
+  mix_fwd_vec_body<T, 32>(H, w, L, n, out, sw);
+}
+template <typename T>
+__global__ __launch_bounds__(1024) void mix_fwd_vec_narrow_kernel(const T* __restrict__ H, const float* __restrict__ w,
+                                                                 int L, long n, T* __restrict__ out) {
+  __shared__ float sw[64];
+  mix_fwd_vec_body<T, 8>(H, w, L, n, out, sw);
+}
+template <typename T>
+__device__ __forceinline__ void mix_bwd_vec_block(const T* __restrict__ H, const T* __restrict__ dOut, int L, long n,
+                                                  float* __restrict__ partial, long b, long nb, int tid, bool active,
+                                                  float (*red)[32]) {
   constexpr int VEC = Elem<T>::VEC;
-  __shared__ float red[4][32];
-  const int lane = threadIdx.x & 63, wave = threadIdx.x >> 6;
+  const int lane = tid & 63, wave = tid >> 6;
   float acc[32];
 #pragma unroll
   for (int l = 0; l < 32; ++l) acc[l] = 0.f;
   const long nv = n / VEC;
-  for (long i = (long)blockIdx.x * blockDim.x + threadIdx.x; i < nv; i += (long)gridDim.x * blockDim.x) {
+  for (long i = active ? b * 256 + tid : nv; i < nv; i += nb * 256) {
     float d[VEC];
     unpack16(*reinterpret_cast<const uint4*>(dOut + i * VEC), d, (const T*)nullptr);
 #pragma unroll
@@ -647,19 +704,39 @@
     if (lane == 0) red[wave][l] = a;
   }
   __syncthreads();
-  if (threadIdx.x < L)
-    partial[(long)blockIdx.x * L + threadIdx.x] =
-        red[0][threadIdx.x] + red[1][threadIdx.x] + red[2][threadIdx.x] + red[3][threadIdx.x];
+  if (active && tid < L) partial[b * L + tid] = red[0][tid] + red[1][tid] + red[2][tid] + red[3][tid];
+}
+template <typename T>
+__global__ __launch_bounds__(256) void mix_bwd_vec_kernel(const T* __restrict__ H, const T* __restrict__ dOut,
+                                                          int L, long n, float* __restrict__ partial) {
+  __shared__ float red[4][32];
+  mix_bwd_vec_block<T>(H, dOut, L, n, partial, blockIdx.x, gridDim.x, threadIdx.x, true, red);
+}
+template <typename T>
+__global__ __launch_bounds__(1024) void mix_bwd_vec_narrow_kernel(const T* __restrict__ H, const T* __restrict__ dOut,
+                                                                 int L, long n, float* __restrict__ partial, long nvb) {
+  __shared__ float red[4][4][32];
+  const int q = tell_quarter();
+  for (long vb0 = (long)blockIdx.x * 4; vb0 < nvb; vb0 += (long)gridDim.x * 4) {
+    mix_bwd_vec_block<T>(H, dOut, L, n, partial, vb0 + q, nvb, threadIdx.x & 255, vb0 + q < nvb, red[q]);
+    __syncthreads();
+  }
 }
 extern "C" int tell_mix_fwd(const void* H, const float* w, int L, long n, void* out, int dtype,
                             hipStream_t stream) {
   TELL_REQUIRE(L >= 1 && L <= 64, "mix_fwd: L must be in [1,64]");
+  const long G = tell_opt(OPT_BW_WGS);
   if (L <= 32 && n % 8 == 0 && (((uintptr_t)H | (uintptr_t)out) & 15) == 0 && dtype == TELL_BF16) {
-    hipLaunchKernelGGL((mix_fwd_vec_kernel<uint16_t>), dim3(grid_for(n / 8, 256)), dim3(256), 0, stream, (const uint16_t*)H, w, L, n, (uint16_t*)out);
+    const int gv = grid_for(n / 8, 256);
+    if (G > 0) tell_launch_narrow(mix_fwd_vec_narrow_kernel<uint16_t>, tell_narrow_wgs(G, gv), 1024, stream, (const uint16_t*)H, w, L, n, (uint16_t*)out);
+    else hipLaunchKernelGGL((mix_fwd_vec_kernel<uint16_t>), dim3(gv), dim3(256), 0, stream, (const uint16_t*)H, w, L, n, (uint16_t*)out);
     return tell_check_launch("mix_fwd_vec");
   }
   int g = grid_for(n, 256 * 4);
-  if (dtype == TELL_BF16) hipLaunchKernelGGL((mix_fwd_kernel<uint16_t>), dim3(g), dim3(256), 0, stream, (const uint16_t*)H, w, L, n, (uint16_t*)out);
+  if (G > 0) {
+    if (dtype == TELL_BF16) tell_launch_narrow(mix_fwd_narrow_kernel<uint16_t>, tell_narrow_wgs(G, g), 1024, stream, (const uint16_t*)H, w, L, n, (uint16_t*)out);
+    else tell_launch_narrow(mix_fwd_narrow_kernel<float>, tell_narrow_wgs(G, g), 1024, stream, (const float*)H, w, L, n, (float*)out);
+  } else if (dtype == TELL_BF16) hipLaunchKernelGGL((mix_fwd_kernel<uint16_t>), dim3(g), dim3(256), 0, stream, (const uint16_t*)H, w, L, n, (uint16_t*)out);
   else hipLaunchKernelGGL((mix_fwd_kernel<float>), dim3(g), dim3(256), 0, stream, (const float*)H, w, L, n, (float*)out);
   return tell_check_launch("mix_fwd");
 }
@@ -667,9 +744,16 @@
                             int n_blocks, int dtype, hipStream_t stream) {
   TELL_REQUIRE(L >= 1 && L <= 64, "mix_bwd: L must be in [1,64]");
   TELL_REQUIRE(n_blocks >= 1, "mix_bwd: n_blocks");
+  const long G = tell_opt(OPT_BW_WGS), nvb = n_blocks;
   if (L <= 32 && n % 8 == 0 && (((uintptr_t)H | (uintptr_t)dOut) & 15) == 0 && dtype == TELL_BF16) {
-    hipLaunchKernelGGL((mix_bwd_vec_kernel<uint16_t>), dim3(n_blocks), dim3(256), 0, stream, (const uint16_t*)H, (const uint16_t*)dOut, L, n, partial);
+    if (G > 0) tell_launch_narrow(mix_bwd_vec_narrow_kernel<uint16_t>, tell_narrow_wgs(G, nvb), 1024, stream, (const uint16_t*)H, (const uint16_t*)dOut, L, n, partial, nvb);
+    else hipLaunchKernelGGL((mix_bwd_vec_kernel<uint16_t>), dim3(n_blocks), dim3(256), 0, stream, (const uint16_t*)H, (const uint16_t*)dOut, L, n, partial);
     return tell_check_launch("mix_bwd_vec");
+  }
+  if (G > 0) {
+    if (dtype == TELL_BF16) tell_launch_narrow(mix_bwd_narrow_kernel<uint16_t>, tell_narrow_wgs(G, nvb), 1024, stream, (const uint16_t*)H, (const uint16_t*)dOut, L, n, partial, nvb);
+    else tell_launch_narrow(mix_bwd_narrow_kernel<float>, tell_narrow_wgs(G, nvb), 1024, stream, (const float*)H, (const float*)dOut, L, n, partial, nvb);
+    return tell_check_launch("mix_bwd");
   }
   if (dtype == TELL_BF16) hipLaunchKernelGGL((mix_bwd_kernel<uint16_t>), dim3(n_blocks), dim3(256), 0, stream, (const uint16_t*)H, (const uint16_t*)dOut, L, n, partial);
   else hipLaunchKernelGGL((mix_bwd_kernel<float>), dim3(n_blocks), dim3(256), 0, stream, (const float*)H, (const float*)dOut, L, n, partial);
diff --git a/transform-and-tell_amd/csrc/optim.hip b/transform-and-tell_amd/csrc/optim.hip
--- a/transform-and-tell_amd/csrc/optim.hip
+++ b/transform-and-tell_amd/csrc/optim.hip
@@ -15,25 +15,43 @@
   return reinterpret_cast<const float4*>(grad)[o];
 }
 template <int U>
+__device__ __forceinline__ void sqsum_chunks_trip(const float* __restrict__ grad, const uint16_t* __restrict__ wire,
+                                                  long n_chunks, float grad_scale, float* __restrict__ partial, long c0,
+                                                  int tid, float (*red)[4]) {
+  float4 g[U];
+#pragma unroll
+  for (int u = 0; u < U; ++u)
+    g[u] = c0 + u < n_chunks ? load_grad4(grad, wire, (c0 + u) * OPT_CHUNK / 4 + tid) : make_float4(0.f, 0.f, 0.f, 0.f);
+#pragma unroll
+  for (int u = 0; u < U; ++u) {
+#pragma clang fp contract(off)
+    float s;
+    if (u == 0) s = ((g[u].x * g[u].x + g[u].y * g[u].y) + g[u].z * g[u].z) + g[u].w * g[u].w;
+    else s = __builtin_fmaf(g[u].w, g[u].w, __builtin_fmaf(g[u].z, g[u].z, __builtin_fmaf(g[u].x, g[u].x, g[u].y * g[u].y)));
+    s = (s * grad_scale) * grad_scale;
+    s = wave_sum(s);
+    if ((tid & 63) == 0) red[u][tid >> 6] = s;
+  }
+  __syncthreads();
+  if (tid < U && c0 + tid < n_chunks) partial[c0 + tid] = red[tid][0] + red[tid][1] + red[tid][2] + red[tid][3];
+  __syncthreads();
+}
+template <int U>
 __global__ __launch_bounds__(256) void sqsum_chunks_kernel(const float* __restrict__ grad, const uint16_t* __restrict__ wire,
                                                            long n_chunks, float grad_scale, float* __restrict__ partial) {
   __shared__ float red[U][4];
-  for (long c0 = (long)blockIdx.x * U; c0 < n_chunks; c0 += (long)gridDim.x * U) {
-    float4 g[U];
-#pragma unroll
-    for (int u = 0; u < U; ++u)
-      g[u] = c0 + u < n_chunks ? load_grad4(grad, wire, (c0 + u) * OPT_CHUNK / 4 + threadIdx.x) : make_float4(0.f, 0.f, 0.f, 0.f);
-#pragma unroll
-    for (int u = 0; u < U; ++u) {
-      float s = (g[u].x * g[u].x + g[u].y * g[u].y + g[u].z * g[u].z + g[u].w * g[u].w) * grad_scale * grad_scale;
-      s = wave_sum(s);
-      if ((threadIdx.x & 63) == 0) red[u][threadIdx.x >> 6] = s;
-    }
-    __syncthreads();
-    if (threadIdx.x < U && c0 + threadIdx.x < n_chunks)
-      partial[c0 + threadIdx.x] = red[threadIdx.x][0] + red[threadIdx.x][1] + red[threadIdx.x][2] + red[threadIdx.x][3];
-    __syncthreads();
-  }
+  for (long c0 = (long)blockIdx.x * U; c0 < n_chunks; c0 += (long)gridDim.x * U)
+    sqsum_chunks_trip<U>(grad, wire, n_chunks, grad_scale, partial, c0, threadIdx.x, red);
+}
+template <int U>
+__global__ __launch_bounds__(1024) void sqsum_chunks_narrow_kernel(const float* __restrict__ grad,
+                                                                   const uint16_t* __restrict__ wire, long n_chunks,
+                                                                   float grad_scale, float* __restrict__ partial, long nvb) {
+  __shared__ float red[4][U][4];
+  const int q = tell_quarter(), tid = threadIdx.x & 255;
+  for (long vb0 = (long)blockIdx.x * 4; vb0 < nvb; vb0 += (long)gridDim.x * 4)
+    for (long c0 = vb0 * U; c0 < n_chunks; c0 += nvb * U)
+      sqsum_chunks_trip<U>(grad, wire, n_chunks, grad_scale, partial, vb0 + q < nvb ? c0 + q * U : n_chunks, tid, red[q]);
 }
 __global__ __launch_bounds__(256) void tensor_norms_kernel(const float* __restrict__ partial,
                                                            const long* __restrict__ chunk_begin,
@@ -107,6 +125,9 @@
   float* ema;
   const float* omd_dev;
 };
+struct NarrowArgs {
+  long nvb;
+};
 template <typename T>
 __device__ __forceinline__ const T* trailing_arg() { return nullptr; }
 template <typename T, typename A, typename... R>
@@ -117,7 +138,7 @@
 template <typename T, typename... Ts>
 constexpr int count_of = (0 + ... + (std::is_same<T, Ts>::value ? 1 : 0));
 template <int U, bool NT, typename... Ext>
-__global__ __launch_bounds__(256) void bertadam_update_kernel(float* __restrict__ param,
+__global__ __launch_bounds__((count_of<NarrowArgs, Ext...> == 1 ? 1024 : 256)) void bertadam_update_kernel(float* __restrict__ param,
                                                               float* __restrict__ grad,
                                                               float* __restrict__ m, float* __restrict__ v,
                                                               const int* __restrict__ chunk_tensor,
@@ -130,15 +151,19 @@
                                                               int* __restrict__ step_dev,
                                                               const int* __restrict__ keep_grad, Ext... ext) {
   constexpr bool EMA = count_of<EmaArgs, Ext...> == 1, GROUPS = count_of<GroupArgs, Ext...> == 1;
-  static_assert(sizeof...(Ext) == (EMA ? 1 : 0) + (GROUPS ? 1 : 0),
-                "the optional trailing arguments are one EmaArgs, one GroupArgs, or both in that order");
+  constexpr bool NARROW = count_of<NarrowArgs, Ext...> == 1;
+  static_assert(sizeof...(Ext) == (NARROW ? 1 : 0) + (EMA ? 1 : 0) + (GROUPS ? 1 : 0),
+                "the optional trailing arguments are one NarrowArgs, one EmaArgs, one GroupArgs, or several in that order");
+  const int tid = NARROW ? threadIdx.x & 255 : threadIdx.x;
+  long vb = NARROW ? (long)blockIdx.x * 4 + tell_quarter() : blockIdx.x, nvb = gridDim.x;
+  if constexpr (NARROW) nvb = trailing_arg<NarrowArgs>(ext...)->nvb;
   typedef __attribute__((ext_vector_type(4))) float f4;
   struct Hp { float lr, b1, b2, eps, wd, max_norm; };
   Hp one = {0.f, b1, b2, eps, wd, max_norm};
   if constexpr (!GROUPS) one.lr = *lr_dev;
   float* ema = nullptr;
   float omd = 0.f;
-  if constexpr (EMA && !GROUPS) {
+  if constexpr (EMA && !GROUPS && !NARROW) {
     const EmaArgs ea[] = {ext...};
     ema = ea[0].ema;
     omd = *ea[0].omd_dev;
@@ -152,9 +177,9 @@
   if (skip && skip[0] != 0) {
     if (blockIdx.x == 0 && threadIdx.x == 0) atomicAdd(skip + 1, 1);
     if (zero_grad)
-      for (long c = blockIdx.x; c < n_chunks; c += gridDim.x)
+      for (long c = vb; c < n_chunks; c += NARROW ? (long)gridDim.x * 4 : nvb)
         if (!keep_grad || !keep_grad[chunk_tensor[c]])
-          reinterpret_cast<float4*>(grad)[c * OPT_CHUNK / 4 + threadIdx.x] = make_float4(0.f, 0.f, 0.f, 0.f);
+          reinterpret_cast<float4*>(grad)[c * OPT_CHUNK / 4 + tid] = make_float4(0.f, 0.f, 0.f, 0.f);
     return;
   }
   if (step_dev && blockIdx.x == 0 && threadIdx.x == 0) atomicAdd(step_dev, 1);
@@ -166,7 +191,9 @@
     f4* q = reinterpret_cast<f4*>(base) + o;
     if (NT) __builtin_nontemporal_store(val, q); else *q = val;
   };
-  for (long c0 = (long)blockIdx.x * U; c0 < n_chunks; c0 += (long)gridDim.x * U) {
+  if (NARROW && vb >= nvb) return;
+  do
+  for (long c0 = vb * U; c0 < n_chunks; c0 += nvb * U) {
     f4 g[U], p[U], mm[U], vv[U], e[EMA ? U : 1];
     float coef[U];
     int tensor[U], group[GROUPS ? U : 1];
@@ -174,7 +201,7 @@
 #pragma unroll
     for (int u = 0; u < U; ++u) {
       const long c = c0 + u < n_chunks ? c0 + u : n_chunks - 1;
-      const long o = c * OPT_CHUNK / 4 + threadIdx.x;
+      const long o = c * OPT_CHUNK / 4 + tid;
       if (wire) { const float4 w = load_grad4(grad, wire, o); g[u] = f4{w.x, w.y, w.z, w.w}; }
       else g[u] = ldf(grad, o);
       p[u] = ldf(param, o); mm[u] = ldf(m, o); vv[u] = ldf(v, o);
@@ -199,7 +226,7 @@
 #pragma unroll
     for (int u = 0; u < U; ++u) {
       if (c0 + u >= n_chunks) break;
-      const long o = (c0 + u) * OPT_CHUNK / 4 + threadIdx.x;
+      const long o = (c0 + u) * OPT_CHUNK / 4 + tid;
       const Hp h = GROUPS ? hp[GROUPS ? u : 0] : one;
       const float lr = h.lr, b1 = h.b1, b2 = h.b2, eps = h.eps, wd = h.wd;
 #pragma unroll
@@ -226,6 +253,7 @@
       if (zero_grad && !(keep_grad && keep_grad[tensor[u]])) stf(grad, o, f4{0.f, 0.f, 0.f, 0.f});
     }
   }
+  while (NARROW && (vb += (long)gridDim.x * 4) < nvb);
 }
 
 __global__ __launch_bounds__(256) void ema_swap_kernel(float* __restrict__ param, float* __restrict__ ema,
@@ -259,6 +287,34 @@
 
 extern "C" int tell_opt_chunk(void) { return OPT_CHUNK; }
 
+struct AdamFixed {
+  float *param, *grad, *m, *v;
+  const int* chunk_tensor;
+  const float* norms;
+  long n_chunks;
+  const float* lr_dev;
+  float b1, b2, eps, wd, max_norm, grad_scale;
+  uint16_t* shadow;
+  int zero_grad;
+  int* skip;
+  const uint16_t* wire;
+  int* step_dev;
+  const int* keep_grad;
+};
+template <int U, bool NT, typename... Ext>
+static void adam_launch(long G, int g, hipStream_t stream, const AdamFixed& f, Ext... ext) {
+  if (G > 0) {
+    void (*kern)(float*, float*, float*, float*, const int*, const float*, long, const float*, float, float, float, float, float,
+                 float, uint16_t*, int, int*, const uint16_t*, int*, const int*, NarrowArgs, Ext...) =
+        bertadam_update_kernel<U, NT, NarrowArgs, Ext...>;
+    tell_launch_narrow(kern, tell_narrow_wgs(G, g), 1024, stream, f.param, f.grad, f.m, f.v, f.chunk_tensor, f.norms, f.n_chunks,
+                       f.lr_dev, f.b1, f.b2, f.eps, f.wd, f.max_norm, f.grad_scale, f.shadow, f.zero_grad, f.skip, f.wire,
+                       f.step_dev, f.keep_grad, NarrowArgs{g}, ext...);
+  } else
+    hipLaunchKernelGGL((bertadam_update_kernel<U, NT, Ext...>), dim3(g), dim3(256), 0, stream, f.param, f.grad, f.m, f.v,
+                       f.chunk_tensor, f.norms, f.n_chunks, f.lr_dev, f.b1, f.b2, f.eps, f.wd, f.max_norm, f.grad_scale,
+                       f.shadow, f.zero_grad, f.skip, f.wire, f.step_dev, f.keep_grad, ext...);
+}
 template <bool EMA>
 static int bertadam_launch(float* param, float* grad, float* m, float* v, const int* chunk_tensor, const long* chunk_begin,
                            long n_chunks, int n_tensors, float* partial, float* norms, const float* lr_dev, float b1, float b2,
@@ -302,30 +358,27 @@
   const int U = (var == 1 || var == 3) ? 2 : (var == 2 || var == 4) ? 4 : 1;
   const long iters = (n_chunks + U - 1) / U;
   int g = iters < grid_env ? (int)iters : grid_env;
+  const long G = tell_opt(OPT_BW_WGS);
   if (max_norm > 0.f) {
     const long it4 = (n_chunks + 3) / 4;
     const int gs = it4 < 4096 ? (int)it4 : 4096;
-    hipLaunchKernelGGL((sqsum_chunks_kernel<4>), dim3(gs), dim3(256), 0, stream, grad, wire, n_chunks, grad_scale, partial);
+    if (G > 0)
+      tell_launch_narrow(sqsum_chunks_narrow_kernel<4>, tell_narrow_wgs(G, gs), 1024, stream, grad, wire, n_chunks, grad_scale,
+                         partial, (long)gs);
+    else
+      hipLaunchKernelGGL((sqsum_chunks_kernel<4>), dim3(gs), dim3(256), 0, stream, grad, wire, n_chunks, grad_scale, partial);
     hipLaunchKernelGGL(tensor_norms_kernel, dim3(n_tensors), dim3(256), 0, stream, partial, chunk_begin, n_tensors, norms, skip);
   }
-#define TELL_ADAM_LAUNCH(UU, NTT)                                                                                               \
-  do {                                                                                                                        \
-    if (EMA && groups)                                                                                                        \
-      hipLaunchKernelGGL((bertadam_update_kernel<UU, NTT, EmaArgs, GroupArgs>), dim3(g), dim3(256), 0, stream, param, grad, m,  \
-                         v, chunk_tensor, norms, n_chunks, lr_dev, 0.f, 0.f, 0.f, 0.f, 0.f, grad_scale,                        \
-                         (uint16_t*)shadow_bf16, zero_grad, skip, wire, step_dev, keep_grad, EmaArgs{ema, omd_dev}, *groups);  \
-    else if (groups)                                                                                                          \
-      hipLaunchKernelGGL((bertadam_update_kernel<UU, NTT, GroupArgs>), dim3(g), dim3(256), 0, stream, param, grad, m, v,        \
-                         chunk_tensor, norms, n_chunks, lr_dev, 0.f, 0.f, 0.f, 0.f, 0.f, grad_scale,                          \
-                         (uint16_t*)shadow_bf16, zero_grad, skip, wire, step_dev, keep_grad, *groups);                         \
-    else if (EMA)                                                                                                             \
-      hipLaunchKernelGGL((bertadam_update_kernel<UU, NTT, EmaArgs>), dim3(g), dim3(256), 0, stream, param, grad, m, v,              \
-                         chunk_tensor, norms, n_chunks, lr_dev, b1, b2, eps, wd, max_norm, grad_scale,                        \
-                         (uint16_t*)shadow_bf16, zero_grad, skip, wire, step_dev, keep_grad, EmaArgs{ema, omd_dev});           \
-    else                                                                                                                      \
-      hipLaunchKernelGGL((bertadam_update_kernel<UU, NTT>), dim3(g), dim3(256), 0, stream, param, grad, m, v, chunk_tensor,   \
-                         norms, n_chunks, lr_dev, b1, b2, eps, wd, max_norm, grad_scale, (uint16_t*)shadow_bf16, zero_grad,   \
-                         skip, wire, step_dev, keep_grad);                                                                    \
+  const AdamFixed f = {param, grad, m, v, chunk_tensor, norms, n_chunks, lr_dev, b1, b2, eps, wd, max_norm, grad_scale,
+                       (uint16_t*)shadow_bf16, zero_grad, skip, wire, step_dev, keep_grad};
+#define TELL_ADAM_LAUNCH(UU, NTT)                                                                          \
+  do {                                                                                                     \
+    AdamFixed fg = f;                                                                                      \
+    fg.max_norm = 0.f;                                                                                     \
+    if (EMA && groups) adam_launch<UU, NTT>(G, g, stream, fg, EmaArgs{ema, omd_dev}, *groups);             \
+    else if (groups) adam_launch<UU, NTT>(G, g, stream, fg, *groups);                                      \
+    else if (EMA) adam_launch<UU, NTT>(G, g, stream, f, EmaArgs{ema, omd_dev});                            \
+    else adam_launch<UU, NTT>(G, g, stream, f);                                                            \
   } while (0)
   switch (var) {
     case 1: TELL_ADAM_LAUNCH(2, false); break;
diff --git a/transform-and-tell_amd/csrc/options.h b/transform-and-tell_amd/csrc/options.h
--- a/transform-and-tell_amd/csrc/options.h
+++ b/transform-and-tell_amd/csrc/options.h
@@ -36,6 +36,7 @@
   X(OPT_ARGMAX_REGS, "argmax_regs", 1)                                                                                  \
   X(OPT_ADAM_VAR, "adam_var", -1)                                                   \
   X(OPT_ADAM_GRID, "adam_grid", 4096)                                                                                   \
+  X(OPT_BW_WGS, "bw_wgs", 0)                \
   X(OPT_SK_ROWS, "sk_rows", 0)              \
   X(OPT_SK_SPLIT, "sk_split", 0)            \
   X(OPT_SK_TALL_WAVES, "sk_tall_waves", 4)                    \
diff --git a/transform-and-tell_amd/training/trainer.py b/transform-and-tell_amd/training/trainer.py
--- a/transform-and-tell_amd/training/trainer.py
+++ b/transform-and-tell_amd/training/trainer.py
@@ -44,6 +44,11 @@
         if self.dp and self.world > 1:
             if 'TELL_Q4_DYNAMIC' not in os.environ:
                 hip.set_option('q4_dynamic', 1)
+        self._lib_options = {}
+        if torch.device(device).type == 'cuda':
+            for key, value in (('bw_wgs', 128), ('q4_dynamic', 1)):
+                if 'TELL_' + key.upper() not in os.environ:
+                    self._lib_options[key] = value
         if self.dp:
             rt.set_rank(self.rank)
         if self.dp:
@@ -141,7 +146,9 @@
     def train_one_batch(self, batch, next_batch=None):
         if self.optimizer.ema_swapped:
             raise RuntimeError('train_one_batch inside Trainer.ema_weights(): the masters sit in the EMA buffer')
-        with hip.bound_stream():
+        overlapped = bool(self._lib_options) and next_batch is not None
+        scoped = hip.options(**self._lib_options) if overlapped else contextlib.nullcontext()
+        with hip.bound_stream(), scoped:
             return self._train_one_batch(batch, next_batch)
 
     def _encoded_for(self, batch):
```

Measured after the change: 1662 samples/s (median of 6 runs). +1.3%, better.
